# ak110/object_detector

Measured on AMD Instinct MI355X. Metric: images_per_sec, higher is better.
Workload: dtype f16

## Files before the change

object_detector_amd/csrc/conv_8ph.hip:

```cpp
#include "conv_common.h"

namespace {

constexpr int E_BN = 256, E_BK = 64;
constexpr int E_REGION = 128 * 128;
constexpr int E_BUF = 4 * E_REGION;
constexpr int E_ALO = 0, E_AHI = E_REGION, E_BLO = 2 * E_REGION, E_BHI = 3 * E_REGION;

struct TapWalk {
  int c0, tap, tapoff, dx;
  int sel_tap;
};

constexpr unsigned E_OOB = 0x80000000u;

template <int MT, int NF = 4, bool KEEP = false>
static __device__ __forceinline__ void e8_epilogue_direct(const ConvKP& p, f32x4 (&acc)[MT][NF], int m0w, int n0w, int l15,
                                                          int lq, f16x8 (*keep)[NF / 2] = nullptr, int mrows = MT * 16,
                                                          const float* pre_sc = nullptr, const float* pre_bi = nullptr) {
  unsigned pb[MT], ppix[MT];
#pragma unroll
  for (int i = 0; i < MT; ++i) {
    const int m = m0w + i * 16 + l15;
    pb[i] = (unsigned)m / (unsigned)p.HoWo;
    ppix[i] = (unsigned)m - pb[i] * (unsigned)p.HoWo;
  }
#pragma unroll
  for (int pr = 0; pr < NF / 2; ++pr) {
    const int n = n0w + (2 * pr + (lq & 1)) * 16 + (lq >> 1) * 8;
    const bool nok = n < p.Cout;
    float sc[8], bi[8];
    if (pre_sc) {
#pragma unroll
      for (int e = 0; e < 8; ++e) {
        sc[e] = pre_sc[e];
        bi[e] = pre_bi[e];
      }
    } else {
      const f32x4 s0 = *(const f32x4*)(p.scale + n), s1 = *(const f32x4*)(p.scale + n + 4);
      const f32x4 b0 = *(const f32x4*)(p.bias + n), b1 = *(const f32x4*)(p.bias + n + 4);
#pragma unroll
      for (int e = 0; e < 4; ++e) {
        sc[e] = s0[e];
        sc[4 + e] = s1[e];
        bi[e] = b0[e];
        bi[4 + e] = b1[e];
      }
    }
    f16x8 rv[MT];
#pragma unroll
    for (int i = 0; i < MT; ++i) {
      const int m = m0w + i * 16 + l15;
      f16x8 r = {0, 0, 0, 0, 0, 0, 0, 0};
      if (nok && m < p.M && p.res_mode != OD_RES_NONE) {
        long long roff;
        if (p.res_mode == OD_RES_SAME) {
          roff = (long long)m * p.Cout + n;
        } else {
          const unsigned ho = ppix[i] / (unsigned)p.Wo, wo = ppix[i] - ho * (unsigned)p.Wo;
          roff = ((long long)(pb[i] * (unsigned)(p.Ho >> 1) + (ho >> 1)) * (p.Wo >> 1) + (wo >> 1)) * p.Cout + n;
        }
        r = *(const f16x8*)(p.res + roff);
      }
      rv[i] = r;
    }
#pragma unroll
    for (int i = 0; i < MT; ++i) {
      const int m = m0w + i * 16 + l15;
      const bool ok = nok && m < p.M && i * 16 + l15 < mrows;
      float v[8];
#pragma unroll
      for (int e = 0; e < 4; ++e) {
        float a = acc[i][2 * pr][e], bq = acc[i][2 * pr + 1][e];
        od_permlane16_swap(a, bq);
        v[e] = a;
        v[4 + e] = bq;
      }
#pragma unroll
      for (int e = 0; e < 8; ++e) v[e] = v[e] * sc[e] + bi[e];
      if (p.act == OD_ACT_LEAKY) {
#pragma unroll
        for (int e = 0; e < 8; ++e) v[e] = od_leaky(v[e], p.alpha);
      } else if (p.act == OD_ACT_ELU) {
#pragma unroll
        for (int e = 0; e < 8; ++e) v[e] = v[e] > 0.f ? v[e] : p.alpha * od_expm1_fast(v[e]);
      }
      if (p.res_mode != OD_RES_NONE) {
#pragma unroll
        for (int e = 0; e < 8; ++e) v[e] += (float)rv[i][e];
      }
      if (ok) {
        const long long ooff = (long long)pb[i] * p.obs + (long long)ppix[i] * p.ops + n;
        if (p.out_f32) {
          float* o = (float*)p.out + ooff;
          *(f32x4*)o = f32x4{v[0], v[1], v[2], v[3]};
          *(f32x4*)(o + 4) = f32x4{v[4], v[5], v[6], v[7]};
        } else {
          f16x8 h;
#pragma unroll
          for (int e = 0; e < 8; ++e) h[e] = (f16)v[e];
          *(f16x8*)((f16*)p.out + ooff) = h;
        }
      }
      if (KEEP) {
        f16x8 h;
#pragma unroll
        for (int e = 0; e < 8; ++e) h[e] = (f16)v[e];
        keep[i][pr] = h;
      }
    }
  }
}

template <int KS, int MF1, bool PW = false, bool SEG = false>
__global__ __launch_bounds__(512, 2) void od_conv_8ph(ConvKP p_in) {
  constexpr int MF0 = 4, MT = MF0 + MF1, WROWS = MT * 16, BM = 2 * WROWS;
  extern __shared__ __attribute__((aligned(16))) char smem[];
  const int tid = threadIdx.x;
  const int lane = tid & 63;
  const int wave = __builtin_amdgcn_readfirstlane(tid >> 6);
  const int wr = wave >> 2, wc = wave & 3;
  const int l15 = lane & 15, lq = lane >> 4;

  int logical;
  {
    const int nt = p_in.mtiles * p_in.ntiles;
    const int pid = p_in.splitk > 1 ? (int)blockIdx.x / p_in.splitk : (int)blockIdx.x;
    const int q = nt >> 3, r = nt & 7, xcd = pid & 7, loc = pid >> 3;
    logical = (xcd < r ? xcd * (q + 1) : r * (q + 1) + (xcd - r) * q) + loc;
  }
  int tm = logical / p_in.ntiles;
  const int tn = logical - tm * p_in.ntiles;
  ConvKP p_seg;
  if (SEG) p_seg = p_in;
  if (SEG && p_in.nseg > 1) {
    int sg = 0;
    if (tm >= p_in.seg_tile0[1]) sg = 1;
    if (p_in.nseg > 2 && tm >= p_in.seg_tile0[2]) sg = 2;
    tm -= p_in.seg_tile0[sg];
    p_seg.x = p_in.seg_x[sg];
    p_seg.out = p_in.seg_out[sg];
    p_seg.H = p_seg.Ho = p_in.seg_H[sg];
    p_seg.W = p_seg.Wo = p_in.seg_W[sg];
    p_seg.HoWo = p_seg.H * p_seg.W;
    p_seg.M = p_in.seg_M[sg];
    p_seg.x_bytes = (unsigned)p_seg.M * (unsigned)p_in.Cin * 2u;
    if (p_in.obs == 0) p_seg.obs = (long long)p_seg.HoWo * p_in.Cout;
  }
  const ConvKP& p = SEG ? p_seg : p_in;
  const int m0 = tm * BM, n0 = tn * E_BN;
  const int nk_all = p.Ktot / E_BK;
  const int ks0 = p.splitk > 1 ? ((int)blockIdx.x % p.splitk) * p.steps_per_split : 0;
  const int nk = p.splitk > 1 ? min(p.steps_per_split, nk_all - ks0) : nk_all;
  if (nk <= 0) return;

  const int rr = tid >> 3;
  const int lc = (tid & 7) ^ (rr & 7);
  int a_base[2][2];
  unsigned a_vmask[2][2];
  unsigned a_sel[2][2];
#pragma unroll
  for (int s = 0; s < 2; ++s)
#pragma unroll
    for (int j = 0; j < 2; ++j) {
      const int m = m0 + j * WROWS + s * 64 + rr;
      a_vmask[s][j] = 0u;
      a_base[s][j] = 0;
      if (m < p.M && (s == 0 || rr < MF1 * 16)) {
        const unsigned b = (unsigned)m / (unsigned)p.HoWo;
        const unsigned pix = (unsigned)m - b * (unsigned)p.HoWo;
        const unsigned ho = pix / (unsigned)p.Wo;
        const unsigned wo = pix - ho * (unsigned)p.Wo;
        const int hi0 = (int)ho * p.stride - p.pad, wi0 = (int)wo * p.stride - p.pad;
        a_base[s][j] = ((((int)b * p.H + hi0 + p.pad) * p.W + wi0 + p.pad) * p.Cin + lc * 8) * 2;
#pragma unroll
        for (int t = 0; t < KS * KS; ++t) {
          const int hi = hi0 + t / KS, wi = wi0 + t % KS;
          if ((unsigned)hi < (unsigned)p.H && (unsigned)wi < (unsigned)p.W) a_vmask[s][j] |= 1u << t;
        }
      }
    }
  int w_off[2][2];
#pragma unroll
  for (int s = 0; s < 2; ++s)
#pragma unroll
    for (int j = 0; j < 2; ++j) {
      const int n = n0 + (2 * j + (rr >> 5)) * 64 + s * 32 + (rr & 31);
      w_off[s][j] = (n * p.Kstride + lc * 8 + ks0 * E_BK) * 2;
    }
  const __amdgpu_buffer_rsrc_t rs_x = __builtin_amdgcn_make_buffer_rsrc(
      (void*)(p.x - (long long)p.pad * (p.W + 1) * p.Cin), 0, (int)(p.x_bytes + (unsigned)(p.pad * (p.W + 1) * p.Cin * 2)),
      0x00020000);
  const __amdgpu_buffer_rsrc_t rs_w = __builtin_amdgcn_make_buffer_rsrc((void*)p.w, 0, (int)p.w_bytes, 0x00020000);
  auto blds16 = [&](const __amdgpu_buffer_rsrc_t& rs, unsigned voff, int soff, char* lptr) {
    __builtin_amdgcn_raw_ptr_buffer_load_lds(rs, (__attribute__((address_space(3))) void*)lptr, 16, (int)voff, soff, 0, 0);
  };

  auto walk_init = [&](TapWalk& w, int kt) {
    const int k0 = kt * E_BK;
    if (KS == 3) {
      w.sel_tap = -1;
      w.tap = k0 / p.Cin;
      w.c0 = k0 - w.tap * p.Cin;
      const int dy = w.tap / 3;
      w.dx = w.tap - dy * 3;
      w.tapoff = (dy * p.W + w.dx) * p.Cin;
    } else {
      w.sel_tap = -1;
      w.tap = 0;
      w.c0 = k0;
      w.dx = 0;
      w.tapoff = 0;
    }
  };
  auto walk_next = [&](TapWalk& w) {
    w.c0 += E_BK;
    if (KS == 3 && w.c0 >= p.Cin) {
      w.c0 = 0;
      ++w.tap;
      if (++w.dx == 3) {
        w.dx = 0;
        w.tapoff += (p.W - 2) * p.Cin;
      } else {
        w.tapoff += p.Cin;
      }
    }
  };
  TapWalk walk_lo, walk_hi;
  walk_init(walk_lo, ks0);
  walk_init(walk_hi, ks0);

  char* const piece = smem + wave * 1024;
  auto stage_a = [&](int s, TapWalk& w, int buf) {
    const int koff = w.tapoff + w.c0;
    char* dst = piece + buf * E_BUF + (s ? E_AHI : E_ALO);
    if (w.sel_tap != w.tap) {
      w.sel_tap = w.tap;
#pragma unroll
      for (int j = 0; j < 2; ++j) a_sel[s][j] = ((a_vmask[s][j] >> w.tap) & 1u) ? (unsigned)a_base[s][j] : E_OOB;
    }
#pragma unroll
    for (int j = 0; j < 2; ++j) blds16(rs_x, a_sel[s][j], koff * 2, dst + j * 8192);
    walk_next(w);
  };
  auto stage_b = [&](int s, int t, int buf) {
    char* dst = piece + buf * E_BUF + (s ? E_BHI : E_BLO);
#pragma unroll
    for (int j = 0; j < 2; ++j) blds16(rs_w, (unsigned)w_off[s][j], t * (E_BK * 2), dst + j * 8192);
  };

  const int w2buf = ((nk - 1) & 1) ^ 1;
  const __amdgpu_buffer_rsrc_t rs_w2 =
      __builtin_amdgcn_make_buffer_rsrc((void*)(PW ? p.w2 : p.w), 0, (int)(PW ? p.w2_bytes : p.w_bytes), 0x00020000);
  auto stage_w2 = [&](int ks) {
#pragma unroll
    for (int h = 0; h < 2; ++h)
      blds16(rs_w2, (unsigned)(((h * 64 + rr) * p.K2stride + lc * 8) * 2), ks * (E_BK * 2),
             piece + w2buf * E_BUF + ks * E_REGION + h * 8192);
  };

  f32x4 acc[MT][4];
#pragma unroll
  for (int i = 0; i < MT; ++i)
#pragma unroll
    for (int j = 0; j < 4; ++j) acc[i][j] = f32x4{0.f, 0.f, 0.f, 0.f};

  stage_a(0, walk_lo, 0);
  stage_b(0, 0, 0);
  stage_b(1, 0, 0);
  stage_a(1, walk_hi, 0);
  if (nk > 1) {
    stage_a(0, walk_lo, 1);
    stage_b(0, 1, 1);
    wait_vmcnt<8>();
  } else {
    wait_vmcnt<0>();
  }
  __builtin_amdgcn_s_barrier();

  const int fa = (wr * 64 + l15) * 128 + ((lq ^ (l15 & 7)) * 16);
  const int fb = (wc * 32 + l15) * 128 + ((lq ^ (l15 & 7)) * 16);

  f16x8 xa[MF0][2], wlo[2][2], whi[2][2];
  auto ldf = [&](f16x8& dst, const char* src) { dst = *(const f16x8*)src; };
  auto mma = [&](f32x4& c, const f16x8& a, const f16x8& b) {
    c = __builtin_amdgcn_mfma_f32_16x16x32_f16(a, b, c, 0, 0, 0);
  };

  auto L0 = [&](int t) {
    const char* cur = smem + (t & 1) * E_BUF;
#pragma unroll
    for (int f = 0; f < 2; ++f)
#pragma unroll
      for (int kh = 0; kh < 2; ++kh) ldf(wlo[f][kh], cur + E_BLO + ((fb + f * 2048) ^ (kh * 64)));
#pragma unroll
    for (int f = 0; f < MF0; ++f)
#pragma unroll
      for (int kh = 0; kh < 2; ++kh) ldf(xa[f][kh], cur + E_ALO + ((fa + f * 2048) ^ (kh * 64)));
    if (t + 1 < nk) {
      stage_b(1, t + 1, (t & 1) ^ 1);
      wait_vmcnt<8>();
    } else if (PW) {
      stage_w2(0);
      wait_vmcnt<2>();
    } else {
      wait_vmcnt<0>();
    }
  };
  auto L1 = [&](int t) {
    const char* cur = smem + (t & 1) * E_BUF;
#pragma unroll
    for (int f = 0; f < 2; ++f)
#pragma unroll
      for (int kh = 0; kh < 2; ++kh) ldf(whi[f][kh], cur + E_BHI + ((fb + f * 2048) ^ (kh * 64)));
    if (t + 1 < nk) {
      stage_a(1, walk_hi, (t & 1) ^ 1);
      wait_vmcnt<8>();
    } else if (PW) {
      stage_w2(1);
    } else {
      wait_vmcnt<0>();
    }
  };
  auto L2 = [&](int t) {
    const char* cur = smem + (t & 1) * E_BUF;
#pragma unroll
    for (int f = 0; f < MF1; ++f)
#pragma unroll
      for (int kh = 0; kh < 2; ++kh) ldf(xa[f][kh], cur + E_AHI + ((fa + f * 2048) ^ (kh * 64)));
    if (t + 2 < nk) stage_a(0, walk_lo, t & 1);
    if (PW && t + 1 == nk) stage_w2(2);
  };
  auto L3 = [&](int t) {
    if (t + 2 < nk) {
      stage_b(0, t + 2, t & 1);
      wait_vmcnt<8>();
    } else if (PW && t + 1 == nk) {
      stage_w2(3);
    } else {
      wait_vmcnt<0>();
    }
  };
  auto M = [&](int ph) {
    __builtin_amdgcn_s_setprio(1);
#pragma unroll
    for (int kh = 0; kh < 2; ++kh)
#pragma unroll
      for (int i = 0; i < ((ph < 2) ? MF0 : MF1); ++i)
#pragma unroll
        for (int j = 0; j < 2; ++j) {
          if (ph == 0) mma(acc[i][j], wlo[j][kh], xa[i][kh]);
          if (ph == 1) mma(acc[i][2 + j], whi[j][kh], xa[i][kh]);
          if (ph == 2) mma(acc[MF0 + i][2 + j], whi[j][kh], xa[i][kh]);
          if (ph == 3) mma(acc[MF0 + i][j], wlo[j][kh], xa[i][kh]);
        }
    __builtin_amdgcn_s_setprio(0);
  };

  if (wr == 0) {
    for (int t = 0; t < nk; ++t) {
      L0(t);
      M(0);
      __builtin_amdgcn_s_barrier();
      L1(t);
      M(1);
      __builtin_amdgcn_s_barrier();
      L2(t);
      M(2);
      __builtin_amdgcn_s_barrier();
      L3(t);
      M(3);
      __builtin_amdgcn_s_barrier();
    }
  } else {
    L0(0);
    __builtin_amdgcn_s_barrier();
    for (int t = 0; t < nk; ++t) {
      M(0);
      L1(t);
      __builtin_amdgcn_s_barrier();
      M(1);
      L2(t);
      __builtin_amdgcn_s_barrier();
      M(2);
      L3(t);
      __builtin_amdgcn_s_barrier();
      M(3);
      if (t + 1 < nk) {
        L0(t + 1);
        __builtin_amdgcn_s_barrier();
      }
    }
  }
  __syncthreads();

  if (PW) {
    const int rg = wave >> 2, cg = wave & 3;
    float sc2[8], bi2[8];
    {
      const int n2 = cg * 32 + (lq & 1) * 16 + (lq >> 1) * 8;
      const f32x4 s0 = *(const f32x4*)(p.scale2 + n2), s1 = *(const f32x4*)(p.scale2 + n2 + 4);
      const f32x4 b0 = *(const f32x4*)(p.bias2 + n2), b1 = *(const f32x4*)(p.bias2 + n2 + 4);
#pragma unroll
      for (int e = 0; e < 4; ++e) {
        sc2[e] = s0[e];
        sc2[4 + e] = s1[e];
        bi2[e] = b0[e];
        bi2[4 + e] = b1[e];
      }
    }
    f16x8 ykeep[MT][2];
    od_mfma_results_ready();
    e8_epilogue_direct<MT, 4, true>(p, acc, m0 + wr * WROWS, n0 + wc * 64, l15, lq, ykeep);
    ConvKP p2 = p;
    p2.scale = p.scale2;
    p2.bias = p.bias2;
    p2.act = p.act2;
    p2.alpha = p.alpha2;
    p2.res_mode = OD_RES_NONE;
    p2.out = (void*)p.out2;
    p2.out_f32 = 0;
    p2.Cout = p.Cout2;
    p2.obs = (long long)p.HoWo * p.Cout2;
    p2.ops = p.Cout2;
    char* const ybuf = smem + (w2buf ^ 1) * E_BUF;
    const char* const wbuf = smem + w2buf * E_BUF;
    const int fy = (rg * 64 + l15) * 128 + ((lq ^ (l15 & 7)) * 16);
    const int fw = (cg * 32 + l15) * 128 + ((lq ^ (l15 & 7)) * 16);
#pragma unroll
    for (int half = 0; half < 2; ++half) {
      if (wr == half) {
#pragma unroll
        for (int i = 0; i < MT; ++i)
#pragma unroll
          for (int pr = 0; pr < 2; ++pr) {
            const int row = i * 16 + l15;
            const int chunk = (2 * pr + (lq & 1)) * 2 + (lq >> 1);
            *(f16x8*)(ybuf + wc * E_REGION + row * 128 + ((chunk ^ (row & 7)) * 16)) = ykeep[i][pr];
          }
      }
      asm volatile("s_waitcnt lgkmcnt(0)" ::: "memory");
      __builtin_amdgcn_s_barrier();
      f32x4 acc2[4][2];
#pragma unroll
      for (int i = 0; i < 4; ++i)
#pragma unroll
        for (int f = 0; f < 2; ++f) acc2[i][f] = f32x4{0.f, 0.f, 0.f, 0.f};
#pragma unroll
      for (int ks = 0; ks < 4; ++ks)
#pragma unroll
        for (int kh = 0; kh < 2; ++kh) {
          f16x8 wf[2], yf[4];
#pragma unroll
          for (int f = 0; f < 2; ++f) wf[f] = *(const f16x8*)(wbuf + ks * E_REGION + ((fw + f * 2048) ^ (kh * 64)));
#pragma unroll
          for (int i = 0; i < 4; ++i) yf[i] = *(const f16x8*)(ybuf + ks * E_REGION + ((fy + i * 2048) ^ (kh * 64)));
#pragma unroll
          for (int i = 0; i < 4; ++i)
#pragma unroll
            for (int f = 0; f < 2; ++f) acc2[i][f] = __builtin_amdgcn_mfma_f32_16x16x32_f16(wf[f], yf[i], acc2[i][f], 0, 0, 0);
        }
      od_mfma_results_ready();
      e8_epilogue_direct<4, 2>(p2, acc2, m0 + half * WROWS + rg * 64, cg * 32, l15, lq, nullptr, WROWS - rg * 64, sc2, bi2);
      if (half == 0) {
        asm volatile("s_waitcnt lgkmcnt(0)" ::: "memory");
        __builtin_amdgcn_s_barrier();
      }
    }
  } else if (p.splitk > 1) {
    conv_epilogue<E_BN, 2, 4, MT, 4, 512>(p, smem, acc, m0, n0, tid, wr, wc, l15, lq);
  } else {
    od_mfma_results_ready();
    e8_epilogue_direct<MT>(p, acc, m0 + wr * WROWS, n0 + wc * 64, l15, lq);
  }
}

struct E8Entry {
  int BM;
  const void* k1;
  const char* name1;
  const void* k1pw;
  const void* k3pw;
  const char* name1pw;
  const char* name3pw;
  const void* k3seg;
  const char* name3seg;
};
#define OD_E8(MF1)                                                                                                   \
  {                                                                                                                  \
    32 * (4 + MF1), (const void*)&od_conv_8ph<1, MF1>, "od_conv_8ph<1, " #MF1 ", false, false>",                     \
        (const void*)&od_conv_8ph<1, MF1, true>, (const void*)&od_conv_8ph<3, MF1, true>,                            \
        "od_conv_8ph<1, " #MF1 ", true, false>", "od_conv_8ph<3, " #MF1 ", true, false>",                            \
        (const void*)&od_conv_8ph<3, MF1, false, true>, "od_conv_8ph<3, " #MF1 ", false, true>"                      \
  }
const E8Entry g_e8[] = {OD_E8(4), OD_E8(3), OD_E8(2), OD_E8(1)};
constexpr int kNumE8 = sizeof(g_e8) / sizeof(g_e8[0]);

}

int od_conv_8ph_num_cfgs() { return kNumE8; }

long od_conv_8ph_tiles(int idx, int M, int Cout) { return (long)od_ceil_div(M, g_e8[idx].BM) * od_ceil_div(Cout, E_BN); }
double od_conv_8ph_tile_cost(int idx, int nk) { return 13.0 + 1.78 * nk * (0.5 + 0.0625 * (g_e8[idx].BM / 32)); }

bool od_conv_8ph_can_fuse_pointwise(const ConvKP& p) { return p.splitk == 1 && p.Cout == E_BN && p.Cout2 == 128; }

bool od_conv_8ph_select(int idx, const ConvKP& p, int ksize, ConvKernelInfo* info) {
  if (idx < 0 || idx >= kNumE8) return false;
  if ((p.Cin & 63) != 0 || p.tconv) return false;
  if (p.x_bytes >= 0x7F000000u || p.w_bytes >= 0x7F000000u || p.x_bytes == 0) return false;
  const E8Entry& e = g_e8[idx];
  const bool pw = p.w2 != nullptr;
  if (p.nseg > 1 && (ksize != 3 || pw || p.stride != 1 || p.res_mode != OD_RES_NONE)) return false;
  const size_t epi = (size_t)(e.BM / 2) * (E_BN + 4) * 4;
  *info = {ksize == 1 ? (pw ? e.k1pw : e.k1) : (pw ? e.k3pw : e.k3seg),
           ksize == 1 ? (pw ? e.name1pw : e.name1) : (pw ? e.name3pw : e.name3seg),
           e.BM, E_BN, E_BK, 512, epi > (size_t)2 * E_BUF ? epi : (size_t)2 * E_BUF};
  return true;
}
```

object_detector_amd/csrc/conv_common.h:

```cpp
#pragma once
#include "common.h"

struct ConvKP {
  const f16* x;
  const f16* w;
  const float* scale;
  const float* bias;
  const f16* res;
  void* out;
  const f16* zero;
  int H, W, Cin, Ho, Wo, Cout;
  int stride, pad;
  int Kstride, Ktot, M, HoWo;
  int act;
  float alpha;
  int res_mode, out_f32;
  long long obs, ops;
  int mtiles, ntiles;
  int splitk, steps_per_split;
  float* ws;
  int Mq;
  int tconv, Hs, Ws;
  unsigned x_bytes, w_bytes;
  float* stats;
  const f16* w2;
  const float* scale2;
  const float* bias2;
  f16* out2;
  int Cout2, act2;
  float alpha2;
  unsigned w2_bytes;
  int K2stride;
  int nseg;
  int seg_tile0[4];
  const f16* seg_x[3];
  void* seg_out[3];
  int seg_H[3], seg_W[3], seg_M[3];
};

static __device__ __forceinline__ void glds16(const void* gptr, void* lptr) {
  __builtin_amdgcn_global_load_lds((const __attribute__((address_space(1))) void*)gptr,
                                   (__attribute__((address_space(3))) void*)lptr, 16, 0, 0);
}

static __device__ __forceinline__ float od_expm1_fast(float v) {
  const float poly = v * (1.f + v * (0.5f + v * (1.f / 6 + v * (1.f / 24 + v * (1.f / 120 + v * (1.f / 720))))));
  return v > -0.25f ? poly : __expf(v) - 1.f;
}

static __device__ __forceinline__ void od_permlane16_swap(float& a, float& b) {
  asm volatile("s_nop 1\n\tv_permlane16_swap_b32 %0, %1\n\ts_nop 1" : "+v"(a), "+v"(b));
}
static __device__ __forceinline__ void od_mfma_results_ready() {
  __builtin_amdgcn_sched_barrier(0);
  asm volatile("s_nop 15\n\ts_nop 15" ::: "memory");
  __builtin_amdgcn_sched_barrier(0);
}

static __device__ __forceinline__ float od_leaky(float v, float alpha) { return fmaxf(v, v * alpha); }

template <int N>
static __device__ __forceinline__ void wait_vmcnt() {
  asm volatile("s_waitcnt vmcnt(%0)" ::"n"(N) : "memory");
}


static __device__ __forceinline__ int od_tconv_pixel(const ConvKP& p, unsigned m, unsigned BM) {
  const unsigned t = m / BM, r = m - t * BM;
  const unsigned cls = t & 3u, idx = (t >> 2) * BM + r;
  if (idx >= (unsigned)p.Mq) return -1;
  const unsigned HsWs = (unsigned)(p.Hs * p.Ws);
  const unsigned b = idx / HsWs, q = idx - b * HsWs;
  const unsigned i = q / (unsigned)p.Ws, j = q - i * (unsigned)p.Ws;
  return (int)(b * (unsigned)p.HoWo + (2u * i + (cls >> 1)) * (unsigned)p.Wo + 2u * j + (cls & 1u));
}

template <int BN, int WM, int WN, int MT, int NTL, int NT = WM * WN * 64, bool STATS = false>
static __device__ __forceinline__ void conv_epilogue(const ConvKP& p, char* smem, f32x4 (&acc)[MT][NTL], int m0, int n0,
                                                     int tid, int wm, int wn, int l15, int lq) {
  constexpr int WTM = MT * 16, WTN = NTL * 16, SLD = BN + 4;
  float* stg = (float*)smem;
  constexpr int CH = BN / 8;
  constexpr int RPP = NT / CH;
  const int c8 = (tid % CH) * 8;
  const int n = n0 + c8;
  float sc[8], bi[8];
  if (!STATS) {
    const f32x4 s0 = *(const f32x4*)(p.scale + n), s1 = *(const f32x4*)(p.scale + n + 4);
    const f32x4 b0 = *(const f32x4*)(p.bias + n), b1 = *(const f32x4*)(p.bias + n + 4);
#pragma unroll
    for (int e = 0; e < 4; ++e) {
      sc[e] = s0[e];
      sc[4 + e] = s1[e];
      bi[e] = b0[e];
      bi[4 + e] = b1[e];
    }
  }
  float st0[STATS ? 8 : 1], st1[STATS ? 8 : 1];
  if (STATS) {
#pragma unroll
    for (int e = 0; e < 8; ++e) st0[e] = st1[e] = 0.f;
  }
  constexpr int NPASS = (WTM + RPP - 1) / RPP;
  constexpr bool RAGGED = (WTM % RPP) != 0;
  f16x8 resv[WM][NPASS];
  if (p.res_mode != OD_RES_NONE && p.splitk <= 1) {
#pragma unroll
    for (int wr = 0; wr < WM; ++wr)
#pragma unroll
      for (int ps = 0; ps < NPASS; ++ps) {
        int m = m0 + wr * WTM + ps * RPP + tid / CH;
        f16x8 r = {0, 0, 0, 0, 0, 0, 0, 0};
        if (RAGGED && ps * RPP + tid / CH >= WTM) m = p.M;
        if (p.tconv && m < p.M) m = od_tconv_pixel(p, (unsigned)m, WM * MT * 16);
        if (m >= 0 && m < p.M && n < p.Cout) {
          long long roff;
          if (p.res_mode == OD_RES_SAME) {
            roff = (long long)m * p.Cout + n;
          } else {
            const unsigned b = (unsigned)m / (unsigned)p.HoWo;
            const unsigned pix = (unsigned)m - b * (unsigned)p.HoWo;
            const unsigned ho = pix / (unsigned)p.Wo, wo = pix - ho * (unsigned)p.Wo;
            roff = ((long long)(b * (unsigned)(p.Ho >> 1) + (ho >> 1)) * (p.Wo >> 1) + (wo >> 1)) * p.Cout + n;
          }
          r = *(const f16x8*)(p.res + roff);
        }
        resv[wr][ps] = r;
      }
  }
#pragma unroll
  for (int wr = 0; wr < WM; ++wr) {
    if (wm == wr) {
#pragma unroll
      for (int j = 0; j < NTL; ++j) {
        const int nl = wn * WTN + j * 16 + lq * 4;
#pragma unroll
        for (int i = 0; i < MT; ++i) *(f32x4*)(stg + (i * 16 + l15) * SLD + nl) = acc[i][j];
      }
    }
    __syncthreads();
    if (p.splitk > 1) {
      float* slab = p.ws + (long long)((int)blockIdx.x % p.splitk) * p.M * p.Cout;
#pragma unroll
      for (int ps = 0; ps < NPASS; ++ps) {
        const int row = ps * RPP + tid / CH;
        const int m = (RAGGED && row >= WTM) ? p.M : m0 + wr * WTM + row;
        if (m < p.M && n < p.Cout) {
          float* o = slab + (long long)m * p.Cout + n;
          *(f32x4*)o = *(const f32x4*)(stg + row * SLD + c8);
          *(f32x4*)(o + 4) = *(const f32x4*)(stg + row * SLD + c8 + 4);
        }
      }
      if (wr + 1 < WM) __syncthreads();
      continue;
    }
#pragma unroll
    for (int ps = 0; ps < NPASS; ++ps) {
      const int row = ps * RPP + tid / CH;
      int m = (RAGGED && row >= WTM) ? p.M : m0 + wr * WTM + row;
      if (p.tconv && m < p.M) m = od_tconv_pixel(p, (unsigned)m, WM * MT * 16);
      if (m >= 0 && m < p.M && n < p.Cout) {
        const f32x4 v0 = *(const f32x4*)(stg + row * SLD + c8);
        const f32x4 v1 = *(const f32x4*)(stg + row * SLD + c8 + 4);
        float v[8] = {v0[0], v0[1], v0[2], v0[3], v1[0], v1[1], v1[2], v1[3]};
        if (!STATS) {
#pragma unroll
          for (int e = 0; e < 8; ++e) v[e] = v[e] * sc[e] + bi[e];
        }
        if (STATS) {
        } else if (p.act == OD_ACT_LEAKY) {
#pragma unroll
          for (int e = 0; e < 8; ++e) v[e] = od_leaky(v[e], p.alpha);
        } else if (p.act == OD_ACT_ELU) {
#pragma unroll
          for (int e = 0; e < 8; ++e) v[e] = v[e] > 0.f ? v[e] : p.alpha * od_expm1_fast(v[e]);
        }
        if (!STATS && p.res_mode != OD_RES_NONE) {
#pragma unroll
          for (int e = 0; e < 8; ++e) v[e] += (float)resv[wr][ps][e];
        }
        const unsigned b = (unsigned)m / (unsigned)p.HoWo;
        const unsigned pix = (unsigned)m - b * (unsigned)p.HoWo;
        const long long ooff = (long long)b * p.obs + (long long)pix * p.ops + n;
        if (p.out_f32) {
          float* o = (float*)p.out + ooff;
          *(f32x4*)o = f32x4{v[0], v[1], v[2], v[3]};
          *(f32x4*)(o + 4) = f32x4{v[4], v[5], v[6], v[7]};
        } else {
          f16x8 h;
#pragma unroll
          for (int e = 0; e < 8; ++e) h[e] = (f16)v[e];
          *(f16x8*)((f16*)p.out + ooff) = h;
          if (STATS) {
#pragma unroll
            for (int e = 0; e < 8; ++e) {
              const float q = (float)h[e];
              st0[e] += q;
              st1[e] += q * q;
            }
          }
        }
      }
    }
    if (wr + 1 < WM) __syncthreads();
  }
  if (STATS) {
    static_assert(CH == 8 || CH == 16 || CH == 32, "BN must be 64, 128 or 256");
#pragma unroll
    for (int off = CH; off < 64; off <<= 1) {
#pragma unroll
      for (int e = 0; e < 8; ++e) {
        st0[e] += __shfl_xor(st0[e], off, 64);
        st1[e] += __shfl_xor(st1[e], off, 64);
      }
    }
    __syncthreads();
    float* red = (float*)smem;
    const int wv = tid >> 6, ln = tid & 63;
    if (ln < CH) {
#pragma unroll
      for (int e = 0; e < 8; ++e) {
        red[(wv * CH + ln) * 16 + e] = st0[e];
        red[(wv * CH + ln) * 16 + 8 + e] = st1[e];
      }
    }
    __syncthreads();
    if (tid < CH && n < p.Cout) {
      float a[8], b[8];
#pragma unroll
      for (int e = 0; e < 8; ++e) a[e] = b[e] = 0.f;
      for (int w2 = 0; w2 < NT / 64; ++w2) {
#pragma unroll
        for (int e = 0; e < 8; ++e) {
          a[e] += red[(w2 * CH + tid) * 16 + e];
          b[e] += red[(w2 * CH + tid) * 16 + 8 + e];
        }
      }
      float* row = p.stats + (long long)(m0 / (WM * WTM)) * 2 * p.Cout;
#pragma unroll
      for (int e = 0; e < 8; ++e) {
        row[n + e] = a[e];
        row[p.Cout + n + e] = b[e];
      }
    }
  }
}

struct ConvKernelInfo {
  const void* fn;
  const char* name;
  int BM, BN, BK, threads;
  size_t lds;
};

int od_conv_igemm_num_cfgs();
bool od_conv_igemm_select(int cfg, int ksize, int Cin, bool want_stats, ConvKernelInfo* info);
int od_conv_finish_prepare(const ConvKP& p, od_launches* L);
int od_conv_8ph_num_cfgs();
long od_conv_8ph_tiles(int idx, int M, int Cout);
double od_conv_8ph_tile_cost(int idx, int nk);
bool od_conv_8ph_can_fuse_pointwise(const ConvKP& p);
bool od_conv_8ph_select(int idx, const ConvKP& p, int ksize, ConvKernelInfo* info);
bool od_tconv_small_supported(const od_conv_desc* d);
int od_tconv_small_prepare(od_ctx* ctx, const od_conv_desc* d, od_launches* L);
bool od_conv_rdirect_supported(const od_conv_desc* d);
int od_conv_rdirect_prepare(od_ctx* ctx, const od_conv_desc* d, od_launches* L);
bool od_conv_stream3_supported(const od_conv_desc* d);
int od_conv_stream3_prepare(od_ctx* ctx, const od_conv_desc* d, od_launches* L);
```

object_detector_amd/csrc/conv_dispatch.hip:

```cpp
#include <string.h>

#include "conv_common.h"

namespace {

int pick_cfg(const od_ctx* ctx, int M, int Cin, int Cout, int ksize, bool e8_ok, bool throughput) {
  const int cus = ctx->num_cu;
  const int cfg_e8 = od_conv_igemm_num_cfgs();
  const bool spec_ok = (Cin % 64) == 0;
  if (Cout <= 64) return (ksize == 3 && od_ceil_div(M, 128) >= 8 * cus) ? 1 : 3;
  const long t128 = (long)od_ceil_div(M, 128) * od_ceil_div(Cout, 128);
  if (ksize == 1) {
    if (!spec_ok) return 3;
    if (M <= 4096) return (M >= 2048 && Cin >= 512) ? 6 : 3;
    if (M <= 16384) return 7;
    if (Cout < 256) return 3;
    if (t128 < cus) return 4;
  }
  if (!spec_ok) return t128 >= 2L * cus ? 0 : 2;
  const int nk = od_ceil_div(ksize * ksize * Cin, 64);
  if (throughput && e8_ok && ksize == 3 && Cout >= 192 && M >= 2048) {
    double best = t128 >= cus ? t128 * (7.5 + 1.07 * nk) * 0.5 : t128 * (10.0 + 0.55 * nk);
    int pick = t128 >= cus ? 4 : (Cout <= 256 ? 7 : 5);
    for (int i = 0; i < od_conv_8ph_num_cfgs(); ++i) {
      const long tiles = od_conv_8ph_tiles(i, M, Cout);
      if (tiles * 3 < cus) continue;
      const double c = (double)tiles * od_conv_8ph_tile_cost(i, nk);
      if (c < 0.95 * best) {
        best = c / 0.95;
        pick = cfg_e8 + i;
      }
    }
    return pick;
  }
  if (t128 >= cus) {
    if (Cout == 128) return 2;
    const double c13 = (double)od_ceil_div((int)t128, 2 * cus) * (7.5 + 1.07 * nk);
    double best = 0.93 * c13;
    int pick = 4;
    for (int i = 0; e8_ok && i < od_conv_8ph_num_cfgs(); ++i) {
      const double c = (double)((od_conv_8ph_tiles(i, M, Cout) + cus - 1) / cus) * od_conv_8ph_tile_cost(i, nk);
      if (c < best) {
        best = c;
        pick = cfg_e8 + i;
      }
    }
    return pick;
  }
  if (Cout <= 256) return M < 2048 ? 3 : 7;
  return (M >= 2048 && 2 * t128 <= cus) ? 7 : 5;
}

int conv_describe(const od_ctx* ctx, const od_conv_desc* d, bool want_stats, od_conv_desc* v, ConvKP* kp) {
  if (d && d->nseg > 1) {
    OD_REQUIRE(d->nseg <= 3, "od_conv2d_fwd: nseg %d > 3", d->nseg);
    OD_REQUIRE(d->ksize == 3 && d->stride == 1 && d->res_mode == OD_RES_NONE && !d->w2 && !want_stats && !d->transposed,
               "od_conv2d_fwd: a grouped launch (nseg > 1) is a 3x3 stride-1 layer without residual / w2 / bn_partials / "
               "transposed mode");
    for (int i = 0; i < d->nseg; ++i)
      OD_REQUIRE(d->seg_x[i] && d->seg_out[i] && d->seg_H[i] > 0 && d->seg_W[i] > 0, "od_conv2d_fwd: segment %d is incomplete", i);
  }
  OD_REQUIRE(ctx && d, "od_conv2d_fwd: null ctx/desc");
  *v = *d;
  const bool grouped = d->nseg > 1;
  if (grouped) {
    v->x = d->seg_x[0];
    v->out = d->seg_out[0];
    v->H = d->seg_H[0];
    v->W = d->seg_W[0];
  }
  d = v;
  OD_REQUIRE(d->x && d->w && d->scale && d->bias && d->out, "od_conv2d_fwd: null tensor");
  OD_REQUIRE(d->ksize == 1 || d->ksize == 3, "od_conv2d_fwd: ksize %d unsupported", d->ksize);
  OD_REQUIRE(d->stride == 1 || d->stride == 2, "od_conv2d_fwd: stride %d unsupported", d->stride);
  OD_REQUIRE(d->B > 0 && d->H > 0 && d->W > 0 && d->Cin > 0 && d->Cout > 0, "od_conv2d_fwd: bad dims");
  OD_REQUIRE(d->Cin % 8 == 0 && d->Cout % 8 == 0, "od_conv2d_fwd: Cin/Cout must be multiples of 8 (got %d/%d)",
             d->Cin, d->Cout);
  OD_REQUIRE(d->res_mode == OD_RES_NONE || d->res, "od_conv2d_fwd: res_mode set but res is null");
  OD_REQUIRE(d->act >= OD_ACT_LINEAR && d->act <= OD_ACT_ELU, "od_conv2d_fwd: bad act");
  OD_REQUIRE(d->act != OD_ACT_LEAKY || (d->alpha >= 0.f && d->alpha <= 1.f), "od_conv2d_fwd: leaky slope must be in [0, 1]");
  ConvKP& p = *kp;
  p.pad = d->ksize / 2;
  p.tconv = d->transposed != 0;
  if (p.tconv)
    OD_REQUIRE(d->ksize == 3 && d->stride == 2 && d->Cin % 64 == 0,
               "od_conv2d_fwd: transposed mode is the backward-data of a 3x3 stride-2 conv (Cin %% 64 == 0)");
  p.H = p.tconv ? 2 * d->H : d->H;
  p.W = p.tconv ? 2 * d->W : d->W;
  p.stride = p.tconv ? 1 : d->stride;
  p.Hs = d->H;
  p.Ws = d->W;
  p.Ho = (p.H + 2 * p.pad - d->ksize) / p.stride + 1;
  p.Wo = (p.W + 2 * p.pad - d->ksize) / p.stride + 1;
  if (d->res_mode == OD_RES_UP2)
    OD_REQUIRE(p.Ho % 2 == 0 && p.Wo % 2 == 0, "od_conv2d_fwd: OD_RES_UP2 needs even output size");
  const long long M64 = (long long)d->B * p.Ho * p.Wo;
  OD_REQUIRE(M64 * d->Cout < (1LL << 31) && (long long)d->B * d->H * d->W * d->Cin < (1LL << 31),
             "od_conv2d_fwd: tensor too large for 32-bit element offsets");
  p.HoWo = p.Ho * p.Wo;
  long long Mg = 0;
  for (int i = 0; grouped && i < d->nseg; ++i) Mg += (long long)d->B * d->seg_H[i] * d->seg_W[i];
  OD_REQUIRE(!grouped || Mg * d->Cout < (1LL << 31), "od_conv2d_fwd: grouped launch too large for 32-bit element offsets");
  p.M = grouped ? (int)Mg : (int)M64;
  p.nseg = grouped ? d->nseg : 0;

  if (want_stats)
    OD_REQUIRE(!p.tconv && d->out_dtype == OD_DT_F16 && d->act == OD_ACT_LINEAR && d->res_mode == OD_RES_NONE,
               "od_conv2d_fwd: bn_partials needs the raw convolution (f16 output, no activation, no residual, no transposed "
               "gather; scale / bias are NOT applied)");
  if (d->w2) {
    OD_REQUIRE(d->scale2 && d->bias2 && d->out2 && d->Cout2 > 0 && d->Cout2 % 8 == 0,
               "od_conv2d_fwd: w2 needs scale2, bias2, out2 and Cout2 (a multiple of 8)");
    OD_REQUIRE(d->act2 >= OD_ACT_LINEAR && d->act2 <= OD_ACT_ELU, "od_conv2d_fwd: bad act2");
    OD_REQUIRE(d->act2 != OD_ACT_LEAKY || (d->alpha2 >= 0.f && d->alpha2 <= 1.f), "od_conv2d_fwd: leaky slope (alpha2) must be in [0, 1]");
    OD_REQUIRE(d->out_dtype == OD_DT_F16 && !p.tconv && !want_stats && d->Cout % 8 == 0 &&
                   (d->out_batch_stride == 0 || d->out_batch_stride == (long long)p.HoWo * d->Cout) &&
                   (d->out_pix_stride == 0 || d->out_pix_stride == d->Cout),
               "od_conv2d_fwd: w2 (the consuming pointwise layer) needs a dense f16 output of the first layer");
  }
  p.x = (const f16*)d->x;
  p.w = (const f16*)d->w;
  p.scale = d->scale;
  p.bias = d->bias;
  p.res = (const f16*)d->res;
  p.out = d->out;
  p.zero = (const f16*)ctx->zero_page;
  p.Cin = d->Cin;
  p.Cout = d->Cout;
  p.Ktot = d->ksize * d->ksize * d->Cin;
  p.Kstride = od_round_up(p.Ktot, 64);
  p.act = d->act;
  p.alpha = d->alpha;
  p.res_mode = d->res_mode;
  p.out_f32 = d->out_dtype == OD_DT_F32;
  p.stats = d->bn_partials;
  p.w2 = nullptr;
  p.scale2 = d->scale2;
  p.bias2 = d->bias2;
  p.out2 = (f16*)d->out2;
  p.Cout2 = d->Cout2;
  p.act2 = d->act2;
  p.alpha2 = d->alpha2;
  p.K2stride = od_round_up(d->Cout, 64);
  p.w2_bytes = (unsigned)((long long)od_round_up(d->Cout2 > 0 ? d->Cout2 : 1, 256) * p.K2stride * 2);
  p.x_bytes = (unsigned)((long long)d->B * d->H * d->W * d->Cin * 2);
  p.w_bytes = (unsigned)((long long)od_round_up(d->Cout, 256) * p.Kstride * 2);
  p.obs = d->out_batch_stride ? d->out_batch_stride : (long long)p.HoWo * d->Cout;
  p.ops = d->out_pix_stride ? d->out_pix_stride : d->Cout;
  p.splitk = 1;
  p.steps_per_split = 0;
  p.ws = (float*)d->splitk_workspace;
  return OD_OK;
}

int conv_choose_cfg(const od_ctx* ctx, const od_conv_desc* d, const ConvKP& p, bool want_stats, int* cfg_out) {
  int cfg = d->tile_cfg;
  if (cfg < 0)
    cfg = pick_cfg(ctx, p.M, d->Cin, d->Cout, d->ksize, !want_stats && !p.tconv && (long long)p.x_bytes < 0x7F000000LL, cfg == -2);
  const int cfg_e8 = od_conv_igemm_num_cfgs();
  OD_REQUIRE(cfg < cfg_e8 + od_conv_8ph_num_cfgs(), "od_conv2d_fwd: tile_cfg %d out of range", cfg);
  OD_REQUIRE(!(want_stats && cfg >= cfg_e8), "od_conv2d_fwd: bn_partials is supported by the table kernels only (tile_cfg %d)", cfg);
  OD_REQUIRE(!p.tconv || cfg < cfg_e8, "od_conv2d_fwd: transposed mode runs on the table kernels only (tile_cfg %d)", cfg);
  *cfg_out = cfg;
  return OD_OK;
}

int conv_select(int cfg, const od_conv_desc* d, const ConvKP& p, bool want_stats, ConvKernelInfo* k) {
  const int cfg_e8 = od_conv_igemm_num_cfgs();
  if (cfg >= cfg_e8) {
    if (od_conv_8ph_select(cfg - cfg_e8, p, d->ksize, k)) return OD_OK;
    od_set_error("od_conv2d_fwd: tile_cfg %d (8-phase kernel) needs Cin %% 64 == 0 and no transposed gather", cfg);
    return OD_ERR_INVALID;
  }
  if (od_conv_igemm_select(cfg, d->ksize, d->Cin, want_stats, k)) return OD_OK;
  od_set_error("od_conv2d_fwd: tile_cfg %d needs Cin %% %d == 0 for 3x3 (Cin = %d); use cfg 0-3", cfg, k->BK, d->Cin);
  return OD_ERR_INVALID;
}

void conv_tile_kp(const od_conv_desc* d, const ConvKernelInfo& k, ConvKP* kp) {
  ConvKP& p = *kp;
  p.mtiles = od_ceil_div(p.M, k.BM);
  if (p.nseg > 1) {
    int t0 = 0;
    for (int i = 0; i < 3; ++i) {
      const bool used = i < d->nseg;
      p.seg_tile0[i] = t0;
      p.seg_x[i] = used ? (const f16*)d->seg_x[i] : nullptr;
      p.seg_out[i] = used ? d->seg_out[i] : nullptr;
      p.seg_H[i] = used ? d->seg_H[i] : 0;
      p.seg_W[i] = used ? d->seg_W[i] : 0;
      p.seg_M[i] = d->B * p.seg_H[i] * p.seg_W[i];
      t0 += od_ceil_div(p.seg_M[i], k.BM);
    }
    p.seg_tile0[3] = t0;
    p.mtiles = t0;
    if (!d->out_batch_stride) p.obs = 0;
  }
  p.Mq = 0;
  if (p.tconv) {
    p.Mq = p.M / 4;
    p.mtiles = 4 * od_ceil_div(p.Mq, k.BM);
    p.M = p.mtiles * k.BM;
  }
  p.ntiles = od_ceil_div(d->Cout, k.BN);
}

int conv_prepare(od_ctx* ctx, const od_conv_desc* desc, bool want_stats, od_launches* L) {
  od_conv_desc v;
  ConvKP p;
  if (int rc = conv_describe(ctx, desc, want_stats, &v, &p)) return rc;
  const od_conv_desc* d = &v;
  const bool grouped = p.nseg > 1;
  if (d->tile_cfg < 0 && !want_stats && !grouped) {
    if (p.tconv && od_tconv_small_supported(d)) return od_tconv_small_prepare(ctx, d, L);
    if (od_conv_rdirect_supported(d)) return od_conv_rdirect_prepare(ctx, d, L);
    if (!p.tconv && od_conv_stream3_supported(d)) return od_conv_stream3_prepare(ctx, d, L);
  }
  int cfg;
  if (int rc = conv_choose_cfg(ctx, d, p, want_stats, &cfg)) return rc;
  const bool use_e8 = cfg >= od_conv_igemm_num_cfgs();
  if (grouped && !(use_e8 && d->Cin % 64 == 0)) {
    od_conv_desc q = *d;
    q.nseg = 0;
    for (int i = 0; i < d->nseg; ++i) {
      q.x = d->seg_x[i];
      q.out = d->seg_out[i];
      q.H = d->seg_H[i];
      q.W = d->seg_W[i];
      if (int rc = conv_prepare(ctx, &q, false, L)) return rc;
    }
    return OD_OK;
  }
  ConvKernelInfo k;
  if (int rc = conv_select(cfg, d, p, want_stats, &k)) return rc;
  conv_tile_kp(d, k, &p);
  if (d->bn_partials) {
    const long long need = (long long)p.mtiles * 2 * d->Cout * 4;
    if (d->bn_partials_bytes < need) {
      od_set_error("od_conv2d_fwd: bn_partials holds %lld bytes, %d rows x 2 x %d channels need %lld", (long long)d->bn_partials_bytes,
                   p.mtiles, d->Cout, need);
      return OD_ERR_WORKSPACE;
    }
  }
  if (d->splitk_workspace && d->splitk != 1 && !p.tconv && !want_stats && !grouped) {
    const int cus = ctx->num_cu;
    const int tiles = p.mtiles * p.ntiles;
    const int nk = od_ceil_div(p.Ktot, k.BK);
    constexpr int thr_mul = 8;
    constexpr int tgt_mul = 1;
    int sk = d->splitk > 1 ? d->splitk : ((tiles * thr_mul <= cus && nk >= 8) ? od_ceil_div(tgt_mul * cus / 2, tiles) : 1);
    if (sk > nk / 4) sk = nk / 4;
    const long long slab_bytes = (long long)p.M * d->Cout * 4;
    if ((long long)sk * slab_bytes > (long long)d->splitk_workspace_bytes) sk = (int)(d->splitk_workspace_bytes / slab_bytes);
    if (sk > 1) {
      p.steps_per_split = od_ceil_div(nk, sk);
      p.splitk = od_ceil_div(nk, p.steps_per_split);
    }
  }
  if (d->w2 && use_e8 && od_conv_8ph_can_fuse_pointwise(p)) {
    p.w2 = (const f16*)d->w2;
    if (int rc = conv_select(cfg, d, p, want_stats, &k)) return rc;
  }
  if (int rc = od_ensure_lds(ctx, k.fn, k.lds)) return rc;
  const size_t launch_lds = (use_e8 && p.splitk <= 1 && k.lds > (size_t)128 * 1024) ? (size_t)128 * 1024 : k.lds;
  if (int rc = od_add_launch(L, {k.name, od_issue_kp, k.fn, dim3(p.mtiles * p.ntiles * p.splitk), dim3(k.threads), launch_lds}, p))
    return rc;
  if (p.splitk > 1)
    if (int rc = od_conv_finish_prepare(p, L)) return rc;
  if (!d->w2 || p.w2) return OD_OK;
  od_conv_desc q;
  memset(&q, 0, sizeof(q));
  q.x = d->out;
  q.w = d->w2;
  q.scale = d->scale2;
  q.bias = d->bias2;
  q.out = d->out2;
  q.B = d->B;
  q.H = p.Ho;
  q.W = p.Wo;
  q.Cin = d->Cout;
  q.Cout = d->Cout2;
  q.ksize = 1;
  q.stride = 1;
  q.act = d->act2;
  q.alpha = d->alpha2;
  q.res_mode = OD_RES_NONE;
  q.out_dtype = OD_DT_F16;
  q.tile_cfg = d->tile_cfg < 0 ? d->tile_cfg : -1;
  q.splitk = d->splitk;
  q.splitk_workspace = d->splitk_workspace;
  q.splitk_workspace_bytes = d->splitk_workspace_bytes;
  return conv_prepare(ctx, &q, false, L);
}

}

extern "C" int od_conv_num_tile_cfgs(void) { return od_conv_igemm_num_cfgs() + od_conv_8ph_num_cfgs(); }

extern "C" int od_conv_weight_dims(int cout, int cin, int ksize, int* cout_pad, int* kpad) {
  OD_REQUIRE(cout > 0 && cin > 0 && (ksize == 1 || ksize == 3), "od_conv_weight_dims: bad dims");
  if (cout_pad) *cout_pad = od_round_up(cout, 256);
  if (kpad) *kpad = od_round_up(ksize * ksize * cin, 64);
  return OD_OK;
}

int od_conv_prepare(od_ctx* ctx, const od_conv_desc* d, od_launches* L) {
  return conv_prepare(ctx, d, d && d->bn_partials, L);
}

extern "C" int od_conv2d_fwd(od_ctx* ctx, const od_conv_desc* d, void* stream) {
  return od_prepare_issue(stream, od_conv_prepare, ctx, d);
}

extern "C" int od_conv2d_fwd_bn_rows(od_ctx* ctx, const od_conv_desc* d) {
  od_conv_desc v;
  ConvKP p;
  ConvKernelInfo k;
  int cfg;
  if (conv_describe(ctx, d, true, &v, &p) || conv_choose_cfg(ctx, &v, p, true, &cfg) || conv_select(cfg, &v, p, true, &k)) return -1;
  conv_tile_kp(&v, k, &p);
  return p.mtiles;
}

extern "C" int od_conv2d_bwd_data(od_ctx* ctx, const void* dz, const void* w_bwd, const void* dx_accumulate, void* dx, int B,
                                  int Ho, int Wo, int Cin, int Cout, int ksize, int stride, void* stream) {
  OD_REQUIRE(ctx && dz && w_bwd && dx, "od_conv2d_bwd_data: null argument");
  OD_REQUIRE(Cin > 0 && Cin <= 2048, "od_conv2d_bwd_data: Cin out of range (1..2048)");
  od_conv_desc d;
  memset(&d, 0, sizeof(d));
  d.x = dz;
  d.w = w_bwd;
  d.scale = ctx->ones;
  d.bias = (const float*)ctx->zero_page;
  d.res = dx_accumulate;
  d.res_mode = dx_accumulate ? OD_RES_SAME : OD_RES_NONE;
  d.out = dx;
  d.B = B;
  d.H = Ho;
  d.W = Wo;
  d.Cin = Cout;
  d.Cout = Cin;
  d.ksize = ksize;
  d.stride = stride;
  d.act = OD_ACT_LINEAR;
  d.out_dtype = OD_DT_F16;
  d.tile_cfg = -1;
  d.transposed = stride == 2;
  d.splitk = 1;
  return od_conv2d_fwd(ctx, &d, stream);
}
```

object_detector_amd/csrc/conv_mfma.hip:

```cpp
#include <stdlib.h>
#include <string.h>

#include "conv_common.h"

namespace {

template <int BM, int BN, int BK, int STAGES, int WM, int WN, int SPEC = 0>
struct ConvCfg {
  static constexpr int NT = WM * WN * 64;
  static constexpr int NTHREADS = NT * (SPEC ? 2 : 1);
  static constexpr int CPR = BK / 8;
  static constexpr int RPR = NT / CPR;
  static constexpr int AR = BM / RPR, BR = BN / RPR;
  static constexpr int ROWB = BK * 2;
  static constexpr int A_BYTES = BM * ROWB, B_BYTES = BN * ROWB, STAGE_BYTES = A_BYTES + B_BYTES;
  static constexpr int WTM = BM / WM, WTN = BN / WN;
  static constexpr int MT = WTM / 16, NTL = WTN / 16;
  static constexpr int SLD = BN + 4;
  static constexpr int PIPE_BYTES = STAGES * STAGE_BYTES;
  static constexpr int EPI_BYTES = WTM * SLD * 4;
  static constexpr int LDS_BYTES = PIPE_BYTES > EPI_BYTES ? PIPE_BYTES : EPI_BYTES;
  static constexpr int LOADS = AR + BR;
  static_assert(BM % RPR == 0 && BN % RPR == 0, "tile must be a whole number of DMA rounds");
  static_assert(BK == 32 || BK == 64, "BK");
  static_assert(LOADS * (STAGES - 2 > 0 ? STAGES - 2 : 0) <= 63, "vmcnt field");
};

template <int BM, int BN, int BK, int STAGES, int WM, int WN, int KS, int MINW, bool UNI, int SPEC, bool STATS = false>
__global__ __launch_bounds__(WM* WN * 64 * (SPEC ? 2 : 1), MINW) void od_conv_igemm(ConvKP p) {
  using Cf = ConvCfg<BM, BN, BK, STAGES, WM, WN, SPEC>;
  constexpr int NT = Cf::NT, AR = Cf::AR, BR = Cf::BR, RPR = Cf::RPR, ROWB = Cf::ROWB;
  constexpr int WTM = Cf::WTM, WTN = Cf::WTN, MT = Cf::MT, NTL = Cf::NTL;

  extern __shared__ __attribute__((aligned(16))) char smem[];

  const int tid_all = threadIdx.x;
  const int lane = tid_all & 63;
  const int wave_all = __builtin_amdgcn_readfirstlane(tid_all >> 6);
  const bool is_loader = SPEC ? (wave_all >= WM * WN) : true;
  const bool is_consumer = SPEC ? (wave_all < WM * WN) : true;
  const int tid = SPEC ? (tid_all & (NT - 1)) : tid_all;
  const int wave = SPEC ? (wave_all >= WM * WN ? wave_all - WM * WN : wave_all) : wave_all;
  const int l15 = lane & 15, lq = lane >> 4;

  int logical;
  {
    const int nt = p.mtiles * p.ntiles;
    const int pid = p.splitk > 1 ? (int)blockIdx.x / p.splitk : (int)blockIdx.x;
    const int q = nt >> 3, r = nt & 7, xcd = pid & 7, loc = pid >> 3;
    logical = (xcd < r ? xcd * (q + 1) : r * (q + 1) + (xcd - r) * q) + loc;
  }
  const int tm = logical / p.ntiles, tn = logical - tm * p.ntiles;
  const int m0 = tm * BM, n0 = tn * BN;
  const int nk_all = (p.Ktot + BK - 1) / BK;
  const int ks0 = p.splitk > 1 ? ((int)blockIdx.x % p.splitk) * p.steps_per_split : 0;
  int nk = p.splitk > 1 ? min(p.steps_per_split, nk_all - ks0) : nk_all;
  if (nk <= 0) return;

  int rr, lc, piece_off;
  if (BK == 64) {
    rr = tid >> 3;
    lc = (tid & 7) ^ (rr & 7);
    piece_off = wave * 8 * ROWB;
  } else {
    rr = wave * 16 + (lane & 15);
    lc = lane >> 4;
    piece_off = wave * 16 * ROWB;
  }
  int a_base[AR], a_hi0[AR], a_wi0[AR], a_b[AR];
  unsigned a_vmask[AR];
#pragma unroll
  for (int rd = 0; rd < AR; ++rd) {
    int m = m0 + rd * RPR + rr;
    a_vmask[rd] = 0u;
    if (p.tconv && m < p.M) m = od_tconv_pixel(p, (unsigned)m, BM);
    if (m >= 0 && m < p.M) {
      const unsigned b = (unsigned)m / (unsigned)p.HoWo;
      const unsigned pix = (unsigned)m - b * (unsigned)p.HoWo;
      const unsigned ho = pix / (unsigned)p.Wo;
      const unsigned wo = pix - ho * (unsigned)p.Wo;
      a_hi0[rd] = (int)ho * p.stride - p.pad;
      a_wi0[rd] = (int)wo * p.stride - p.pad;
      a_base[rd] = (((int)b * p.H + a_hi0[rd]) * p.W + a_wi0[rd]) * p.Cin + lc * 8;
      a_b[rd] = (int)b;
#pragma unroll
      for (int t = 0; t < KS * KS; ++t) {
        const int hi = a_hi0[rd] + t / KS, wi = a_wi0[rd] + t % KS;
        bool ok = (unsigned)hi < (unsigned)p.H && (unsigned)wi < (unsigned)p.W;
        if (p.tconv) ok = ok && !((hi | wi) & 1);
        if (ok) a_vmask[rd] |= 1u << t;
      }
    } else {
      a_hi0[rd] = -(1 << 24);
      a_wi0[rd] = 0;
      a_base[rd] = 0;
      a_b[rd] = 0;
    }
  }
  const f16* wrow = p.w + (long long)(n0 + rr) * p.Kstride + lc * 8;

  unsigned tmask = 0x1FFu;
  if (UNI && KS == 3 && p.tconv && p.splitk <= 1) {
    unsigned um = 0u;
#pragma unroll
    for (int rd = 0; rd < AR; ++rd) um |= a_vmask[rd];
    for (int off = 32; off; off >>= 1) um |= (unsigned)__shfl_xor((int)um, off, 64);
    unsigned* sh = (unsigned*)smem;
    if (tid_all == 0) *sh = 0u;
    __syncthreads();
    if (lane == 0) atomicOr(sh, um);
    __syncthreads();
    tmask = (unsigned)__builtin_amdgcn_readfirstlane((int)*sh);
    __syncthreads();
    nk = __builtin_popcount(tmask) * (p.Cin / BK);
  }

  int ld_k0 = ks0 * BK, ld_c0 = ld_k0, ld_tap = 0, ld_tapoff = 0, ld_dx = 0, ld_dy = 0;
  if (UNI && KS == 3) {
    ld_tap = ld_k0 / p.Cin;
    ld_c0 = ld_k0 - ld_tap * p.Cin;
    if (tmask != 0x1FFu && tmask != 0u) {
      ld_tap = __builtin_ctz(tmask);
      ld_c0 = 0;
      ld_k0 = ld_tap * p.Cin;
    }
    ld_dy = ld_tap / 3;
    ld_dx = ld_tap - ld_dy * 3;
    ld_tapoff = (ld_dy * p.W + ld_dx) * p.Cin;
  }

  constexpr int NX = AR + BR;
  f16x8 rtmp[SPEC == 2 ? NX : 1];
  char* rdst[SPEC == 2 ? NX : 1];
  int rn = 0;
  auto xfer = [&](const f16* src, char* lds_piece) {
    if (SPEC == 2) {
      rtmp[rn] = *(const f16x8*)src;
      rdst[rn] = lds_piece + lane * 16;
      ++rn;
    } else {
      glds16(src, lds_piece);
    }
  };
  auto stage = [&](int buf) {
    rn = 0;
    char* abuf = smem + buf * Cf::STAGE_BYTES + piece_off;
    char* bbuf = abuf + Cf::A_BYTES;
    if (UNI) {
      const bool cvalid = (KS == 3) || (ld_c0 + lc * 8 < p.Cin);
      const int koff = ld_tapoff + ld_c0;
#pragma unroll
      for (int rd = 0; rd < AR; ++rd) {
        const bool ok = cvalid && ((a_vmask[rd] >> ld_tap) & 1u);
        const f16* src;
        if (KS == 3 && p.tconv) {
          const int u = (a_hi0[rd] + ld_dy) >> 1, v = (a_wi0[rd] + ld_dx) >> 1;
          src = ok ? p.x + (((a_b[rd] * p.Hs + u) * p.Ws + v) * p.Cin + lc * 8 + ld_c0) : p.zero;
        } else {
          src = ok ? p.x + (a_base[rd] + koff) : p.zero;
        }
        xfer(src, abuf + rd * RPR * ROWB);
      }
    } else {
      const int k = ld_k0 + lc * 8;
      const int tap = k / p.Cin;
      const int dy = tap / 3, dx = tap - dy * 3;
      const int cin = k - tap * p.Cin;
      const bool kvalid = k < p.Ktot;
      const int koff = (dy * p.W + dx) * p.Cin + cin - lc * 8;
#pragma unroll
      for (int rd = 0; rd < AR; ++rd) {
        const int hi = a_hi0[rd] + dy, wi = a_wi0[rd] + dx;
        const bool ok = kvalid && (unsigned)hi < (unsigned)p.H && (unsigned)wi < (unsigned)p.W;
        const f16* src = ok ? p.x + (a_base[rd] + koff) : p.zero;
        xfer(src, abuf + rd * RPR * ROWB);
      }
    }
#pragma unroll
    for (int rd = 0; rd < BR; ++rd) xfer(wrow + (long long)rd * RPR * p.Kstride + ld_k0, bbuf + rd * RPR * ROWB);
    if (SPEC == 2) {
#pragma unroll
      for (int i = 0; i < NX; ++i) *(f16x8*)rdst[i] = rtmp[i];
    }
    ld_k0 += BK;
    if (UNI) {
      ld_c0 += BK;
      if (KS == 3 && ld_c0 >= p.Cin) {
        ld_c0 = 0;
        ++ld_tap;
        if (++ld_dx == 3) {
          ld_dx = 0;
          ++ld_dy;
          ld_tapoff += (p.W - 2) * p.Cin;
        } else {
          ld_tapoff += p.Cin;
        }
        while (ld_tap < 9 && !((tmask >> ld_tap) & 1u)) {
          ++ld_tap;
          ld_k0 += p.Cin;
          if (++ld_dx == 3) {
            ld_dx = 0;
            ++ld_dy;
          }
        }
      }
    }
  };

  const int wm = wave / WN, wn = wave - wm * WN;
  f32x4 acc[MT][NTL];
#pragma unroll
  for (int i = 0; i < MT; ++i)
#pragma unroll
    for (int j = 0; j < NTL; ++j) acc[i][j] = f32x4{0.f, 0.f, 0.f, 0.f};

  if (is_loader) {
#pragma unroll
    for (int s = 0; s < STAGES - 1; ++s)
      if (s < nk) stage(s);
  }

  const int swz = l15 & 7;
  int buf = 0;
  for (int ks = 0; ks < nk; ++ks) {
    if (is_loader) {
      if (STAGES > 2 && ks + (STAGES - 2) < nk)
        wait_vmcnt<Cf::LOADS*(STAGES > 2 ? STAGES - 2 : 0)>();
      else
        wait_vmcnt<0>();
    }
    if (SPEC == 2) asm volatile("s_waitcnt lgkmcnt(0)" ::: "memory");
    __builtin_amdgcn_s_barrier();
    {
      const int nxt = ks + STAGES - 1;
      int nb = buf + STAGES - 1;
      if (nb >= STAGES) nb -= STAGES;
      if (is_loader && nxt < nk) stage(nb);
    }
    const char* abuf = smem + buf * Cf::STAGE_BYTES;
    const char* bbuf = abuf + Cf::A_BYTES;
    __builtin_amdgcn_s_setprio(1);
    if (is_consumer)
#pragma unroll
    for (int kh = 0; kh < BK / 32; ++kh) {
      f16x8 xa[MT], wb[NTL];
      if (BK == 64) {
        const int coff = ((kh * 4 + lq) ^ swz) * 16;
#pragma unroll
        for (int i = 0; i < MT; ++i) xa[i] = *(const f16x8*)(abuf + (wm * WTM + i * 16 + l15) * ROWB + coff);
#pragma unroll
        for (int j = 0; j < NTL; ++j) wb[j] = *(const f16x8*)(bbuf + (wn * WTN + j * 16 + l15) * ROWB + coff);
      } else {
        const int coff = lq * 256 + l15 * 16;
#pragma unroll
        for (int i = 0; i < MT; ++i) xa[i] = *(const f16x8*)(abuf + (wm * WTM + i * 16) * ROWB + coff);
#pragma unroll
        for (int j = 0; j < NTL; ++j) wb[j] = *(const f16x8*)(bbuf + (wn * WTN + j * 16) * ROWB + coff);
      }
#pragma unroll
      for (int i = 0; i < MT; ++i)
#pragma unroll
        for (int j = 0; j < NTL; ++j)
          acc[i][j] = __builtin_amdgcn_mfma_f32_16x16x32_f16(wb[j], xa[i], acc[i][j], 0, 0, 0);
    }
    __builtin_amdgcn_s_setprio(0);
    if (++buf == STAGES) buf = 0;
  }
  __syncthreads();

  conv_epilogue<BN, WM, WN, MT, NTL, Cf::NTHREADS, STATS>(p, smem, acc, m0, n0, tid_all, is_consumer ? wm : -1, wn, l15, lq);
}

__global__ __launch_bounds__(256) void od_conv_finish(ConvKP p) {
  const long long nvec = (long long)p.M * (p.Cout >> 3);
  const int C8 = p.Cout >> 3;
  for (long long i = (long long)blockIdx.x * 256 + threadIdx.x; i < nvec; i += (long long)gridDim.x * 256) {
    const int m = (int)(i / C8), n = (int)(i - (long long)m * C8) * 8;
    const float* wsp = p.ws + (long long)m * p.Cout + n;
    const long long slab = (long long)p.M * p.Cout;
    float v[8] = {0.f, 0.f, 0.f, 0.f, 0.f, 0.f, 0.f, 0.f};
    for (int sidx = 0; sidx < p.splitk; ++sidx) {
      const f32x4 a0 = *(const f32x4*)(wsp + sidx * slab), a1 = *(const f32x4*)(wsp + sidx * slab + 4);
#pragma unroll
      for (int e = 0; e < 4; ++e) {
        v[e] += a0[e];
        v[4 + e] += a1[e];
      }
    }
#pragma unroll
    for (int e = 0; e < 8; ++e) {
      v[e] = v[e] * p.scale[n + e] + p.bias[n + e];
      if (p.act == OD_ACT_LEAKY) v[e] = od_leaky(v[e], p.alpha);
      else if (p.act == OD_ACT_ELU) v[e] = v[e] > 0.f ? v[e] : p.alpha * od_expm1_fast(v[e]);
    }
    const unsigned b = (unsigned)m / (unsigned)p.HoWo;
    const unsigned pix = (unsigned)m - b * (unsigned)p.HoWo;
    if (p.res_mode != OD_RES_NONE) {
      long long roff;
      if (p.res_mode == OD_RES_SAME) {
        roff = (long long)m * p.Cout + n;
      } else {
        const unsigned ho = pix / (unsigned)p.Wo, wo = pix - ho * (unsigned)p.Wo;
        roff = ((long long)(b * (unsigned)(p.Ho >> 1) + (ho >> 1)) * (p.Wo >> 1) + (wo >> 1)) * p.Cout + n;
      }
      const f16x8 r = *(const f16x8*)(p.res + roff);
#pragma unroll
      for (int e = 0; e < 8; ++e) v[e] += (float)r[e];
    }
    const long long ooff = (long long)b * p.obs + (long long)pix * p.ops + n;
    if (p.out_f32) {
      float* o = (float*)p.out + ooff;
      *(f32x4*)o = f32x4{v[0], v[1], v[2], v[3]};
      *(f32x4*)(o + 4) = f32x4{v[4], v[5], v[6], v[7]};
    } else {
      f16x8 h;
#pragma unroll
      for (int e = 0; e < 8; ++e) h[e] = (f16)v[e];
      *(f16x8*)((f16*)p.out + ooff) = h;
    }
  }
}

struct TileCfg {
  int BM, BN, BK, threads;
  size_t lds;
  struct { const void* fn; const char* name; } k[3][2];
};

#define OD_K1(BM, BN, BK, ST, WM, WN, KS, MINW, UNI, SPEC, STATS)                                                       \
  {(const void*)&od_conv_igemm<BM, BN, BK, ST, WM, WN, KS, MINW, UNI, SPEC, STATS>,                                     \
   "od_conv_igemm<" #BM ", " #BN ", " #BK ", " #ST ", " #WM ", " #WN ", " #KS ", " #MINW ", " #UNI ", " #SPEC ", " #STATS ">"}
#define OD_K(BM, BN, BK, ST, WM, WN, KS, MINW, UNI, SPEC)                                                              \
  {OD_K1(BM, BN, BK, ST, WM, WN, KS, MINW, UNI, SPEC, false), OD_K1(BM, BN, BK, ST, WM, WN, KS, MINW, UNI, SPEC, true)}
#define OD_NOK(BM, BN, BK, ST, WM, WN, KS, MINW, UNI, SPEC) {}
#define OD_CFG(BM, BN, BK, ST, WM, WN, MINW, SPEC, K3G)                                                                 \
  {BM, BN, BK, WM * WN * 64 * (SPEC + 1), (size_t)ConvCfg<BM, BN, BK, ST, WM, WN, SPEC>::LDS_BYTES,                     \
   {OD_K(BM, BN, BK, ST, WM, WN, 1, MINW, true, SPEC), OD_K(BM, BN, BK, ST, WM, WN, 3, MINW, true, SPEC),               \
    K3G(BM, BN, BK, ST, WM, WN, 3, MINW, false, SPEC)}}

const TileCfg g_cfgs[] = {
    OD_CFG(128, 128, 64, 2, 2, 2, 2, 0, OD_K),
    OD_CFG(128, 64, 64, 2, 2, 2, 2, 0, OD_K),
    OD_CFG(64, 128, 64, 2, 2, 2, 2, 0, OD_K),
    OD_CFG(64, 64, 64, 2, 2, 2, 2, 0, OD_K),
    OD_CFG(128, 128, 64, 2, 2, 2, 4, 1, OD_NOK),
    OD_CFG(128, 128, 64, 3, 2, 2, 2, 1, OD_NOK),
    OD_CFG(64, 64, 64, 4, 2, 2, 2, 0, OD_NOK),
    OD_CFG(64, 128, 64, 3, 2, 2, 4, 1, OD_NOK),
};
constexpr int kNumCfgs = sizeof(g_cfgs) / sizeof(g_cfgs[0]);

}

int od_conv_igemm_num_cfgs() { return kNumCfgs; }

bool od_conv_igemm_select(int cfg, int ksize, int Cin, bool want_stats, ConvKernelInfo* info) {
  if (cfg < 0 || cfg >= kNumCfgs) return false;
  const TileCfg& tc = g_cfgs[cfg];
  const auto& k = tc.k[ksize == 1 ? 0 : ((Cin % tc.BK) == 0 ? 1 : 2)][want_stats];
  *info = {k.fn, k.name, tc.BM, tc.BN, tc.BK, tc.threads, tc.lds};
  return k.fn != nullptr;
}

int od_conv_finish_prepare(const ConvKP& p, od_launches* L) {
  const long long nvec = (long long)p.M * (p.Cout / 8);
  long long fb = (nvec + 255) / 256;
  if (fb > 2048) fb = 2048;
  return od_add_launch(L, {"od_conv_finish", od_issue_kp, (const void*)&od_conv_finish, dim3((unsigned)fb), dim3(256), 0}, p);
}
```

Before: 21570.

## Specialize conv epilogues at compile time by activation/residual mode with 32-bit offsets

Adds an EPI template parameter so conv kernels are instantiated for the common activation, residual and output-type combinations, and the dispatcher picks a specialized kernel per layer. This removes runtime branches on act, res_mode and out_f32 in the epilogue. It also computes a flag that allows 32-bit output offset arithmetic when the output fits. The 8-phase kernel moves into a header with per-MF variant selectors. In exchange there are many more kernel instantiations, which raises compile time and binary size.

```diff
diff --git a/object_detector_amd/csrc/conv_8ph.hip b/object_detector_amd/csrc/conv_8ph.hip
--- a/object_detector_amd/csrc/conv_8ph.hip
+++ b/object_detector_amd/csrc/conv_8ph.hip
@@ -1,499 +1,14 @@
+#include "conv_8ph_tile.h"
 #include "conv_common.h"
 
 namespace {
 
-constexpr int E_BN = 256, E_BK = 64;
-constexpr int E_REGION = 128 * 128;
-constexpr int E_BUF = 4 * E_REGION;
-constexpr int E_ALO = 0, E_AHI = E_REGION, E_BLO = 2 * E_REGION, E_BHI = 3 * E_REGION;
-
-struct TapWalk {
-  int c0, tap, tapoff, dx;
-  int sel_tap;
-};
-
-constexpr unsigned E_OOB = 0x80000000u;
-
-template <int MT, int NF = 4, bool KEEP = false>
-static __device__ __forceinline__ void e8_epilogue_direct(const ConvKP& p, f32x4 (&acc)[MT][NF], int m0w, int n0w, int l15,
-                                                          int lq, f16x8 (*keep)[NF / 2] = nullptr, int mrows = MT * 16,
-                                                          const float* pre_sc = nullptr, const float* pre_bi = nullptr) {
-  unsigned pb[MT], ppix[MT];
-#pragma unroll
-  for (int i = 0; i < MT; ++i) {
-    const int m = m0w + i * 16 + l15;
-    pb[i] = (unsigned)m / (unsigned)p.HoWo;
-    ppix[i] = (unsigned)m - pb[i] * (unsigned)p.HoWo;
-  }
-#pragma unroll
-  for (int pr = 0; pr < NF / 2; ++pr) {
-    const int n = n0w + (2 * pr + (lq & 1)) * 16 + (lq >> 1) * 8;
-    const bool nok = n < p.Cout;
-    float sc[8], bi[8];
-    if (pre_sc) {
-#pragma unroll
-      for (int e = 0; e < 8; ++e) {
-        sc[e] = pre_sc[e];
-        bi[e] = pre_bi[e];
-      }
-    } else {
-      const f32x4 s0 = *(const f32x4*)(p.scale + n), s1 = *(const f32x4*)(p.scale + n + 4);
-      const f32x4 b0 = *(const f32x4*)(p.bias + n), b1 = *(const f32x4*)(p.bias + n + 4);
-#pragma unroll
-      for (int e = 0; e < 4; ++e) {
-        sc[e] = s0[e];
-        sc[4 + e] = s1[e];
-        bi[e] = b0[e];
-        bi[4 + e] = b1[e];
-      }
-    }
-    f16x8 rv[MT];
-#pragma unroll
-    for (int i = 0; i < MT; ++i) {
-      const int m = m0w + i * 16 + l15;
-      f16x8 r = {0, 0, 0, 0, 0, 0, 0, 0};
-      if (nok && m < p.M && p.res_mode != OD_RES_NONE) {
-        long long roff;
-        if (p.res_mode == OD_RES_SAME) {
-          roff = (long long)m * p.Cout + n;
-        } else {
-          const unsigned ho = ppix[i] / (unsigned)p.Wo, wo = ppix[i] - ho * (unsigned)p.Wo;
-          roff = ((long long)(pb[i] * (unsigned)(p.Ho >> 1) + (ho >> 1)) * (p.Wo >> 1) + (wo >> 1)) * p.Cout + n;
-        }
-        r = *(const f16x8*)(p.res + roff);
-      }
-      rv[i] = r;
-    }
-#pragma unroll
-    for (int i = 0; i < MT; ++i) {
-      const int m = m0w + i * 16 + l15;
-      const bool ok = nok && m < p.M && i * 16 + l15 < mrows;
-      float v[8];
-#pragma unroll
-      for (int e = 0; e < 4; ++e) {
-        float a = acc[i][2 * pr][e], bq = acc[i][2 * pr + 1][e];
-        od_permlane16_swap(a, bq);
-        v[e] = a;
-        v[4 + e] = bq;
-      }
-#pragma unroll
-      for (int e = 0; e < 8; ++e) v[e] = v[e] * sc[e] + bi[e];
-      if (p.act == OD_ACT_LEAKY) {
-#pragma unroll
-        for (int e = 0; e < 8; ++e) v[e] = od_leaky(v[e], p.alpha);
-      } else if (p.act == OD_ACT_ELU) {
-#pragma unroll
-        for (int e = 0; e < 8; ++e) v[e] = v[e] > 0.f ? v[e] : p.alpha * od_expm1_fast(v[e]);
-      }
-      if (p.res_mode != OD_RES_NONE) {
-#pragma unroll
-        for (int e = 0; e < 8; ++e) v[e] += (float)rv[i][e];
-      }
-      if (ok) {
-        const long long ooff = (long long)pb[i] * p.obs + (long long)ppix[i] * p.ops + n;
-        if (p.out_f32) {
-          float* o = (float*)p.out + ooff;
-          *(f32x4*)o = f32x4{v[0], v[1], v[2], v[3]};
-          *(f32x4*)(o + 4) = f32x4{v[4], v[5], v[6], v[7]};
-        } else {
-          f16x8 h;
-#pragma unroll
-          for (int e = 0; e < 8; ++e) h[e] = (f16)v[e];
-          *(f16x8*)((f16*)p.out + ooff) = h;
-        }
-      }
-      if (KEEP) {
-        f16x8 h;
-#pragma unroll
-        for (int e = 0; e < 8; ++e) h[e] = (f16)v[e];
-        keep[i][pr] = h;
-      }
-    }
-  }
-}
-
-template <int KS, int MF1, bool PW = false, bool SEG = false>
-__global__ __launch_bounds__(512, 2) void od_conv_8ph(ConvKP p_in) {
-  constexpr int MF0 = 4, MT = MF0 + MF1, WROWS = MT * 16, BM = 2 * WROWS;
-  extern __shared__ __attribute__((aligned(16))) char smem[];
-  const int tid = threadIdx.x;
-  const int lane = tid & 63;
-  const int wave = __builtin_amdgcn_readfirstlane(tid >> 6);
-  const int wr = wave >> 2, wc = wave & 3;
-  const int l15 = lane & 15, lq = lane >> 4;
-
-  int logical;
-  {
-    const int nt = p_in.mtiles * p_in.ntiles;
-    const int pid = p_in.splitk > 1 ? (int)blockIdx.x / p_in.splitk : (int)blockIdx.x;
-    const int q = nt >> 3, r = nt & 7, xcd = pid & 7, loc = pid >> 3;
-    logical = (xcd < r ? xcd * (q + 1) : r * (q + 1) + (xcd - r) * q) + loc;
-  }
-  int tm = logical / p_in.ntiles;
-  const int tn = logical - tm * p_in.ntiles;
-  ConvKP p_seg;
-  if (SEG) p_seg = p_in;
-  if (SEG && p_in.nseg > 1) {
-    int sg = 0;
-    if (tm >= p_in.seg_tile0[1]) sg = 1;
-    if (p_in.nseg > 2 && tm >= p_in.seg_tile0[2]) sg = 2;
-    tm -= p_in.seg_tile0[sg];
-    p_seg.x = p_in.seg_x[sg];
-    p_seg.out = p_in.seg_out[sg];
-    p_seg.H = p_seg.Ho = p_in.seg_H[sg];
-    p_seg.W = p_seg.Wo = p_in.seg_W[sg];
-    p_seg.HoWo = p_seg.H * p_seg.W;
-    p_seg.M = p_in.seg_M[sg];
-    p_seg.x_bytes = (unsigned)p_seg.M * (unsigned)p_in.Cin * 2u;
-    if (p_in.obs == 0) p_seg.obs = (long long)p_seg.HoWo * p_in.Cout;
-  }
-  const ConvKP& p = SEG ? p_seg : p_in;
-  const int m0 = tm * BM, n0 = tn * E_BN;
-  const int nk_all = p.Ktot / E_BK;
-  const int ks0 = p.splitk > 1 ? ((int)blockIdx.x % p.splitk) * p.steps_per_split : 0;
-  const int nk = p.splitk > 1 ? min(p.steps_per_split, nk_all - ks0) : nk_all;
-  if (nk <= 0) return;
-
-  const int rr = tid >> 3;
-  const int lc = (tid & 7) ^ (rr & 7);
-  int a_base[2][2];
-  unsigned a_vmask[2][2];
-  unsigned a_sel[2][2];
-#pragma unroll
-  for (int s = 0; s < 2; ++s)
-#pragma unroll
-    for (int j = 0; j < 2; ++j) {
-      const int m = m0 + j * WROWS + s * 64 + rr;
-      a_vmask[s][j] = 0u;
-      a_base[s][j] = 0;
-      if (m < p.M && (s == 0 || rr < MF1 * 16)) {
-        const unsigned b = (unsigned)m / (unsigned)p.HoWo;
-        const unsigned pix = (unsigned)m - b * (unsigned)p.HoWo;
-        const unsigned ho = pix / (unsigned)p.Wo;
-        const unsigned wo = pix - ho * (unsigned)p.Wo;
-        const int hi0 = (int)ho * p.stride - p.pad, wi0 = (int)wo * p.stride - p.pad;
-        a_base[s][j] = ((((int)b * p.H + hi0 + p.pad) * p.W + wi0 + p.pad) * p.Cin + lc * 8) * 2;
-#pragma unroll
-        for (int t = 0; t < KS * KS; ++t) {
-          const int hi = hi0 + t / KS, wi = wi0 + t % KS;
-          if ((unsigned)hi < (unsigned)p.H && (unsigned)wi < (unsigned)p.W) a_vmask[s][j] |= 1u << t;
-        }
-      }
-    }
-  int w_off[2][2];
-#pragma unroll
-  for (int s = 0; s < 2; ++s)
-#pragma unroll
-    for (int j = 0; j < 2; ++j) {
-      const int n = n0 + (2 * j + (rr >> 5)) * 64 + s * 32 + (rr & 31);
-      w_off[s][j] = (n * p.Kstride + lc * 8 + ks0 * E_BK) * 2;
-    }
-  const __amdgpu_buffer_rsrc_t rs_x = __builtin_amdgcn_make_buffer_rsrc(
-      (void*)(p.x - (long long)p.pad * (p.W + 1) * p.Cin), 0, (int)(p.x_bytes + (unsigned)(p.pad * (p.W + 1) * p.Cin * 2)),
-      0x00020000);
-  const __amdgpu_buffer_rsrc_t rs_w = __builtin_amdgcn_make_buffer_rsrc((void*)p.w, 0, (int)p.w_bytes, 0x00020000);
-  auto blds16 = [&](const __amdgpu_buffer_rsrc_t& rs, unsigned voff, int soff, char* lptr) {
-    __builtin_amdgcn_raw_ptr_buffer_load_lds(rs, (__attribute__((address_space(3))) void*)lptr, 16, (int)voff, soff, 0, 0);
-  };
-
-  auto walk_init = [&](TapWalk& w, int kt) {
-    const int k0 = kt * E_BK;
-    if (KS == 3) {
-      w.sel_tap = -1;
-      w.tap = k0 / p.Cin;
-      w.c0 = k0 - w.tap * p.Cin;
-      const int dy = w.tap / 3;
-      w.dx = w.tap - dy * 3;
-      w.tapoff = (dy * p.W + w.dx) * p.Cin;
-    } else {
-      w.sel_tap = -1;
-      w.tap = 0;
-      w.c0 = k0;
-      w.dx = 0;
-      w.tapoff = 0;
-    }
-  };
-  auto walk_next = [&](TapWalk& w) {
-    w.c0 += E_BK;
-    if (KS == 3 && w.c0 >= p.Cin) {
-      w.c0 = 0;
-      ++w.tap;
-      if (++w.dx == 3) {
-        w.dx = 0;
-        w.tapoff += (p.W - 2) * p.Cin;
-      } else {
-        w.tapoff += p.Cin;
-      }
-    }
-  };
-  TapWalk walk_lo, walk_hi;
-  walk_init(walk_lo, ks0);
-  walk_init(walk_hi, ks0);
-
-  char* const piece = smem + wave * 1024;
-  auto stage_a = [&](int s, TapWalk& w, int buf) {
-    const int koff = w.tapoff + w.c0;
-    char* dst = piece + buf * E_BUF + (s ? E_AHI : E_ALO);
-    if (w.sel_tap != w.tap) {
-      w.sel_tap = w.tap;
-#pragma unroll
-      for (int j = 0; j < 2; ++j) a_sel[s][j] = ((a_vmask[s][j] >> w.tap) & 1u) ? (unsigned)a_base[s][j] : E_OOB;
-    }
-#pragma unroll
-    for (int j = 0; j < 2; ++j) blds16(rs_x, a_sel[s][j], koff * 2, dst + j * 8192);
-    walk_next(w);
-  };
-  auto stage_b = [&](int s, int t, int buf) {
-    char* dst = piece + buf * E_BUF + (s ? E_BHI : E_BLO);
-#pragma unroll
-    for (int j = 0; j < 2; ++j) blds16(rs_w, (unsigned)w_off[s][j], t * (E_BK * 2), dst + j * 8192);
-  };
-
-  const int w2buf = ((nk - 1) & 1) ^ 1;
-  const __amdgpu_buffer_rsrc_t rs_w2 =
-      __builtin_amdgcn_make_buffer_rsrc((void*)(PW ? p.w2 : p.w), 0, (int)(PW ? p.w2_bytes : p.w_bytes), 0x00020000);
-  auto stage_w2 = [&](int ks) {
-#pragma unroll
-    for (int h = 0; h < 2; ++h)
-      blds16(rs_w2, (unsigned)(((h * 64 + rr) * p.K2stride + lc * 8) * 2), ks * (E_BK * 2),
-             piece + w2buf * E_BUF + ks * E_REGION + h * 8192);
-  };
-
-  f32x4 acc[MT][4];
-#pragma unroll
-  for (int i = 0; i < MT; ++i)
-#pragma unroll
-    for (int j = 0; j < 4; ++j) acc[i][j] = f32x4{0.f, 0.f, 0.f, 0.f};
-
-  stage_a(0, walk_lo, 0);
-  stage_b(0, 0, 0);
-  stage_b(1, 0, 0);
-  stage_a(1, walk_hi, 0);
-  if (nk > 1) {
-    stage_a(0, walk_lo, 1);
-    stage_b(0, 1, 1);
-    wait_vmcnt<8>();
-  } else {
-    wait_vmcnt<0>();
-  }
-  __builtin_amdgcn_s_barrier();
-
-  const int fa = (wr * 64 + l15) * 128 + ((lq ^ (l15 & 7)) * 16);
-  const int fb = (wc * 32 + l15) * 128 + ((lq ^ (l15 & 7)) * 16);
-
-  f16x8 xa[MF0][2], wlo[2][2], whi[2][2];
-  auto ldf = [&](f16x8& dst, const char* src) { dst = *(const f16x8*)src; };
-  auto mma = [&](f32x4& c, const f16x8& a, const f16x8& b) {
-    c = __builtin_amdgcn_mfma_f32_16x16x32_f16(a, b, c, 0, 0, 0);
-  };
-
-  auto L0 = [&](int t) {
-    const char* cur = smem + (t & 1) * E_BUF;
-#pragma unroll
-    for (int f = 0; f < 2; ++f)
-#pragma unroll
-      for (int kh = 0; kh < 2; ++kh) ldf(wlo[f][kh], cur + E_BLO + ((fb + f * 2048) ^ (kh * 64)));
-#pragma unroll
-    for (int f = 0; f < MF0; ++f)
-#pragma unroll
-      for (int kh = 0; kh < 2; ++kh) ldf(xa[f][kh], cur + E_ALO + ((fa + f * 2048) ^ (kh * 64)));
-    if (t + 1 < nk) {
-      stage_b(1, t + 1, (t & 1) ^ 1);
-      wait_vmcnt<8>();
-    } else if (PW) {
-      stage_w2(0);
-      wait_vmcnt<2>();
-    } else {
-      wait_vmcnt<0>();
-    }
-  };
-  auto L1 = [&](int t) {
-    const char* cur = smem + (t & 1) * E_BUF;
-#pragma unroll
-    for (int f = 0; f < 2; ++f)
-#pragma unroll
-      for (int kh = 0; kh < 2; ++kh) ldf(whi[f][kh], cur + E_BHI + ((fb + f * 2048) ^ (kh * 64)));
-    if (t + 1 < nk) {
-      stage_a(1, walk_hi, (t & 1) ^ 1);
-      wait_vmcnt<8>();
-    } else if (PW) {
-      stage_w2(1);
-    } else {
-      wait_vmcnt<0>();
-    }
-  };
-  auto L2 = [&](int t) {
-    const char* cur = smem + (t & 1) * E_BUF;
-#pragma unroll
-    for (int f = 0; f < MF1; ++f)
-#pragma unroll
-      for (int kh = 0; kh < 2; ++kh) ldf(xa[f][kh], cur + E_AHI + ((fa + f * 2048) ^ (kh * 64)));
-    if (t + 2 < nk) stage_a(0, walk_lo, t & 1);
-    if (PW && t + 1 == nk) stage_w2(2);
-  };
-  auto L3 = [&](int t) {
-    if (t + 2 < nk) {
-      stage_b(0, t + 2, t & 1);
-      wait_vmcnt<8>();
-    } else if (PW && t + 1 == nk) {
-      stage_w2(3);
-    } else {
-      wait_vmcnt<0>();
-    }
-  };
-  auto M = [&](int ph) {
-    __builtin_amdgcn_s_setprio(1);
-#pragma unroll
-    for (int kh = 0; kh < 2; ++kh)
-#pragma unroll
-      for (int i = 0; i < ((ph < 2) ? MF0 : MF1); ++i)
-#pragma unroll
-        for (int j = 0; j < 2; ++j) {
-          if (ph == 0) mma(acc[i][j], wlo[j][kh], xa[i][kh]);
-          if (ph == 1) mma(acc[i][2 + j], whi[j][kh], xa[i][kh]);
-          if (ph == 2) mma(acc[MF0 + i][2 + j], whi[j][kh], xa[i][kh]);
-          if (ph == 3) mma(acc[MF0 + i][j], wlo[j][kh], xa[i][kh]);
-        }
-    __builtin_amdgcn_s_setprio(0);
-  };
-
-  if (wr == 0) {
-    for (int t = 0; t < nk; ++t) {
-      L0(t);
-      M(0);
-      __builtin_amdgcn_s_barrier();
-      L1(t);
-      M(1);
-      __builtin_amdgcn_s_barrier();
-      L2(t);
-      M(2);
-      __builtin_amdgcn_s_barrier();
-      L3(t);
-      M(3);
-      __builtin_amdgcn_s_barrier();
-    }
-  } else {
-    L0(0);
-    __builtin_amdgcn_s_barrier();
-    for (int t = 0; t < nk; ++t) {
-      M(0);
-      L1(t);
-      __builtin_amdgcn_s_barrier();
-      M(1);
-      L2(t);
-      __builtin_amdgcn_s_barrier();
-      M(2);
-      L3(t);
-      __builtin_amdgcn_s_barrier();
-      M(3);
-      if (t + 1 < nk) {
-        L0(t + 1);
-        __builtin_amdgcn_s_barrier();
-      }
-    }
-  }
-  __syncthreads();
-
-  if (PW) {
-    const int rg = wave >> 2, cg = wave & 3;
-    float sc2[8], bi2[8];
-    {
-      const int n2 = cg * 32 + (lq & 1) * 16 + (lq >> 1) * 8;
-      const f32x4 s0 = *(const f32x4*)(p.scale2 + n2), s1 = *(const f32x4*)(p.scale2 + n2 + 4);
-      const f32x4 b0 = *(const f32x4*)(p.bias2 + n2), b1 = *(const f32x4*)(p.bias2 + n2 + 4);
-#pragma unroll
-      for (int e = 0; e < 4; ++e) {
-        sc2[e] = s0[e];
-        sc2[4 + e] = s1[e];
-        bi2[e] = b0[e];
-        bi2[4 + e] = b1[e];
-      }
-    }
-    f16x8 ykeep[MT][2];
-    od_mfma_results_ready();
-    e8_epilogue_direct<MT, 4, true>(p, acc, m0 + wr * WROWS, n0 + wc * 64, l15, lq, ykeep);
-    ConvKP p2 = p;
-    p2.scale = p.scale2;
-    p2.bias = p.bias2;
-    p2.act = p.act2;
-    p2.alpha = p.alpha2;
-    p2.res_mode = OD_RES_NONE;
-    p2.out = (void*)p.out2;
-    p2.out_f32 = 0;
-    p2.Cout = p.Cout2;
-    p2.obs = (long long)p.HoWo * p.Cout2;
-    p2.ops = p.Cout2;
-    char* const ybuf = smem + (w2buf ^ 1) * E_BUF;
-    const char* const wbuf = smem + w2buf * E_BUF;
-    const int fy = (rg * 64 + l15) * 128 + ((lq ^ (l15 & 7)) * 16);
-    const int fw = (cg * 32 + l15) * 128 + ((lq ^ (l15 & 7)) * 16);
-#pragma unroll
-    for (int half = 0; half < 2; ++half) {
-      if (wr == half) {
-#pragma unroll
-        for (int i = 0; i < MT; ++i)
-#pragma unroll
-          for (int pr = 0; pr < 2; ++pr) {
-            const int row = i * 16 + l15;
-            const int chunk = (2 * pr + (lq & 1)) * 2 + (lq >> 1);
-            *(f16x8*)(ybuf + wc * E_REGION + row * 128 + ((chunk ^ (row & 7)) * 16)) = ykeep[i][pr];
-          }
-      }
-      asm volatile("s_waitcnt lgkmcnt(0)" ::: "memory");
-      __builtin_amdgcn_s_barrier();
-      f32x4 acc2[4][2];
-#pragma unroll
-      for (int i = 0; i < 4; ++i)
-#pragma unroll
-        for (int f = 0; f < 2; ++f) acc2[i][f] = f32x4{0.f, 0.f, 0.f, 0.f};
-#pragma unroll
-      for (int ks = 0; ks < 4; ++ks)
-#pragma unroll
-        for (int kh = 0; kh < 2; ++kh) {
-          f16x8 wf[2], yf[4];
-#pragma unroll
-          for (int f = 0; f < 2; ++f) wf[f] = *(const f16x8*)(wbuf + ks * E_REGION + ((fw + f * 2048) ^ (kh * 64)));
-#pragma unroll
-          for (int i = 0; i < 4; ++i) yf[i] = *(const f16x8*)(ybuf + ks * E_REGION + ((fy + i * 2048) ^ (kh * 64)));
-#pragma unroll
-          for (int i = 0; i < 4; ++i)
-#pragma unroll
-            for (int f = 0; f < 2; ++f) acc2[i][f] = __builtin_amdgcn_mfma_f32_16x16x32_f16(wf[f], yf[i], acc2[i][f], 0, 0, 0);
-        }
-      od_mfma_results_ready();
-      e8_epilogue_direct<4, 2>(p2, acc2, m0 + half * WROWS + rg * 64, cg * 32, l15, lq, nullptr, WROWS - rg * 64, sc2, bi2);
-      if (half == 0) {
-        asm volatile("s_waitcnt lgkmcnt(0)" ::: "memory");
-        __builtin_amdgcn_s_barrier();
-      }
-    }
-  } else if (p.splitk > 1) {
-    conv_epilogue<E_BN, 2, 4, MT, 4, 512>(p, smem, acc, m0, n0, tid, wr, wc, l15, lq);
-  } else {
-    od_mfma_results_ready();
-    e8_epilogue_direct<MT>(p, acc, m0 + wr * WROWS, n0 + wc * 64, l15, lq);
-  }
-}
-
 struct E8Entry {
   int BM;
-  const void* k1;
-  const char* name1;
-  const void* k1pw;
-  const void* k3pw;
-  const char* name1pw;
-  const char* name3pw;
-  const void* k3seg;
-  const char* name3seg;
+  bool (*variant)(int ksize, bool pw, int epi, int epi2, const void** fn, const char** name);
 };
-#define OD_E8(MF1)                                                                                                   \
-  {                                                                                                                  \
-    32 * (4 + MF1), (const void*)&od_conv_8ph<1, MF1>, "od_conv_8ph<1, " #MF1 ", false, false>",                     \
-        (const void*)&od_conv_8ph<1, MF1, true>, (const void*)&od_conv_8ph<3, MF1, true>,                            \
-        "od_conv_8ph<1, " #MF1 ", true, false>", "od_conv_8ph<3, " #MF1 ", true, false>",                            \
-        (const void*)&od_conv_8ph<3, MF1, false, true>, "od_conv_8ph<3, " #MF1 ", false, true>"                      \
-  }
-const E8Entry g_e8[] = {OD_E8(4), OD_E8(3), OD_E8(2), OD_E8(1)};
+const E8Entry g_e8[] = {{256, od_conv_8ph_variant_mf4}, {224, od_conv_8ph_variant_mf3}, {192, od_conv_8ph_variant_mf2},
+                        {160, od_conv_8ph_variant_mf1}};
 constexpr int kNumE8 = sizeof(g_e8) / sizeof(g_e8[0]);
 
 }
@@ -513,8 +28,13 @@
   const bool pw = p.w2 != nullptr;
   if (p.nseg > 1 && (ksize != 3 || pw || p.stride != 1 || p.res_mode != OD_RES_NONE)) return false;
   const size_t epi = (size_t)(e.BM / 2) * (E_BN + 4) * 4;
-  *info = {ksize == 1 ? (pw ? e.k1pw : e.k1) : (pw ? e.k3pw : e.k3seg),
-           ksize == 1 ? (pw ? e.name1pw : e.name1) : (pw ? e.name3pw : e.name3seg),
-           e.BM, E_BN, E_BK, 512, epi > (size_t)2 * E_BUF ? epi : (size_t)2 * E_BUF};
+  const int epi1 = od_epi_of(p);
+  const int epi2 = (pw && epi1 != OD_EPI_RT) ? od_epi(p.act2, OD_RES_NONE, false) : OD_EPI_RT;
+  const void* fn;
+  const char* name;
+  if (!e.variant(ksize, pw, epi1, epi2, &fn, &name) &&
+      !e.variant(ksize, pw, OD_EPI_RT, OD_EPI_RT, &fn, &name))
+    return false;
+  *info = {fn, name, e.BM, E_BN, E_BK, 512, epi > (size_t)2 * E_BUF ? epi : (size_t)2 * E_BUF};
   return true;
 }
diff --git a/object_detector_amd/csrc/conv_8ph_inst.hip b/object_detector_amd/csrc/conv_8ph_inst.hip
--- /dev/null
+++ b/object_detector_amd/csrc/conv_8ph_inst.hip
@@ -0,0 +1,51 @@
+#include "conv_8ph_kernel.h"
+
+#ifndef OD_E8_MF1
+#error "compile with -DOD_E8_MF1=1..4"
+#endif
+
+namespace {
+
+struct E8Variant {
+  int ksize;
+  bool pw;
+  int epi, epi2;
+  const void* fn;
+  const char* name;
+};
+#define OD_E8V(KS, PW, SEG, EPI, EPI2)                                                                                  \
+  {KS, PW, EPI, EPI2, (const void*)&od_conv_8ph<KS, OD_E8_MF1, EPI, EPI2, PW, SEG>,                                     \
+   "od_conv_8ph<" #KS ", " OD_STR(OD_E8_MF1) ", " OD_STR(EPI) ", " OD_STR(EPI2) ", " #PW ", " #SEG ">"}
+const E8Variant g_variants[] = {
+    OD_E8V(1, false, false, OD_EPI_RT, OD_EPI_RT),
+    OD_E8V(1, false, false, OD_EPI_LEAKY_NONE_F16, OD_EPI_RT),
+    OD_E8V(1, false, false, OD_EPI_ELU_NONE_F16, OD_EPI_RT),
+    OD_E8V(1, false, false, OD_EPI_ELU_UP2_F16, OD_EPI_RT),
+    OD_E8V(1, false, false, OD_EPI_ELU_NONE_F32, OD_EPI_RT),
+    OD_E8V(3, false, true, OD_EPI_RT, OD_EPI_RT),
+    OD_E8V(3, false, true, OD_EPI_LEAKY_NONE_F16, OD_EPI_RT),
+    OD_E8V(3, false, true, OD_EPI_LEAKY_SAME_F16, OD_EPI_RT),
+    OD_E8V(3, false, true, OD_EPI_ELU_NONE_F16, OD_EPI_RT),
+    OD_E8V(3, false, true, OD_EPI_ELU_UP2_F16, OD_EPI_RT),
+    OD_E8V(3, false, true, OD_EPI_LINEAR_NONE_F32, OD_EPI_RT),
+    OD_E8V(3, false, true, OD_EPI_LEAKY_NONE_F32, OD_EPI_RT),
+    OD_E8V(3, false, true, OD_EPI_ELU_NONE_F32, OD_EPI_RT),
+    OD_E8V(1, true, false, OD_EPI_RT, OD_EPI_RT),
+    OD_E8V(3, true, false, OD_EPI_RT, OD_EPI_RT),
+    OD_E8V(3, true, false, OD_EPI_LEAKY_NONE_F16, OD_EPI_LEAKY_NONE_F16),
+    OD_E8V(3, true, false, OD_EPI_LEAKY_SAME_F16, OD_EPI_LEAKY_NONE_F16),
+};
+
+}
+
+#define OD_CAT_(a, b) a##b
+#define OD_CAT(a, b) OD_CAT_(a, b)
+bool OD_CAT(od_conv_8ph_variant_mf, OD_E8_MF1)(int ksize, bool pw, int epi, int epi2, const void** fn, const char** name) {
+  for (const E8Variant& v : g_variants)
+    if (v.ksize == ksize && v.pw == pw && v.epi == epi && v.epi2 == epi2) {
+      *fn = v.fn;
+      *name = v.name;
+      return true;
+    }
+  return false;
+}
diff --git a/object_detector_amd/csrc/conv_8ph_kernel.h b/object_detector_amd/csrc/conv_8ph_kernel.h
--- /dev/null
+++ b/object_detector_amd/csrc/conv_8ph_kernel.h
@@ -0,0 +1,571 @@
+#pragma once
+#include "conv_8ph_tile.h"
+#include "conv_common.h"
+
+namespace {
+
+constexpr int E_ALO = 0, E_AHI = E_REGION, E_BLO = 2 * E_REGION, E_BHI = 3 * E_REGION;
+
+struct TapWalk {
+  int c0, tap, tapoff, dx;
+  int sel_tap;
+};
+
+constexpr unsigned E_OOB = 0x80000000u;
+
+template <int MT, int NF = 4, bool KEEP = false>
+static __device__ __forceinline__ void e8_epilogue_rt(const ConvKP& p, f32x4 (&acc)[MT][NF], int m0w, int n0w, int l15,
+                                                          int lq, f16x8 (*keep)[NF / 2] = nullptr, int mrows = MT * 16,
+                                                          const float* pre_sc = nullptr, const float* pre_bi = nullptr) {
+  unsigned pb[MT], ppix[MT];
+#pragma unroll
+  for (int i = 0; i < MT; ++i) {
+    const int m = m0w + i * 16 + l15;
+    pb[i] = (unsigned)m / (unsigned)p.HoWo;
+    ppix[i] = (unsigned)m - pb[i] * (unsigned)p.HoWo;
+  }
+#pragma unroll
+  for (int pr = 0; pr < NF / 2; ++pr) {
+    const int n = n0w + (2 * pr + (lq & 1)) * 16 + (lq >> 1) * 8;
+    const bool nok = n < p.Cout;
+    float sc[8], bi[8];
+    if (pre_sc) {
+#pragma unroll
+      for (int e = 0; e < 8; ++e) {
+        sc[e] = pre_sc[e];
+        bi[e] = pre_bi[e];
+      }
+    } else {
+      const f32x4 s0 = *(const f32x4*)(p.scale + n), s1 = *(const f32x4*)(p.scale + n + 4);
+      const f32x4 b0 = *(const f32x4*)(p.bias + n), b1 = *(const f32x4*)(p.bias + n + 4);
+#pragma unroll
+      for (int e = 0; e < 4; ++e) {
+        sc[e] = s0[e];
+        sc[4 + e] = s1[e];
+        bi[e] = b0[e];
+        bi[4 + e] = b1[e];
+      }
+    }
+    f16x8 rv[MT];
+#pragma unroll
+    for (int i = 0; i < MT; ++i) {
+      const int m = m0w + i * 16 + l15;
+      f16x8 r = {0, 0, 0, 0, 0, 0, 0, 0};
+      if (nok && m < p.M && p.res_mode != OD_RES_NONE) {
+        long long roff;
+        if (p.res_mode == OD_RES_SAME) {
+          roff = (long long)m * p.Cout + n;
+        } else {
+          const unsigned ho = ppix[i] / (unsigned)p.Wo, wo = ppix[i] - ho * (unsigned)p.Wo;
+          roff = ((long long)(pb[i] * (unsigned)(p.Ho >> 1) + (ho >> 1)) * (p.Wo >> 1) + (wo >> 1)) * p.Cout + n;
+        }
+        r = *(const f16x8*)(p.res + roff);
+      }
+      rv[i] = r;
+    }
+#pragma unroll
+    for (int i = 0; i < MT; ++i) {
+      const int m = m0w + i * 16 + l15;
+      const bool ok = nok && m < p.M && i * 16 + l15 < mrows;
+      float v[8];
+#pragma unroll
+      for (int e = 0; e < 4; ++e) {
+        float a = acc[i][2 * pr][e], bq = acc[i][2 * pr + 1][e];
+        od_permlane16_swap(a, bq);
+        v[e] = a;
+        v[4 + e] = bq;
+      }
+#pragma unroll
+      for (int e = 0; e < 8; ++e) v[e] = v[e] * sc[e] + bi[e];
+      if (p.act == OD_ACT_LEAKY) {
+#pragma unroll
+        for (int e = 0; e < 8; ++e) v[e] = od_leaky(v[e], p.alpha);
+      } else if (p.act == OD_ACT_ELU) {
+#pragma unroll
+        for (int e = 0; e < 8; ++e) v[e] = v[e] > 0.f ? v[e] : p.alpha * od_expm1_fast(v[e]);
+      }
+      if (p.res_mode != OD_RES_NONE) {
+#pragma unroll
+        for (int e = 0; e < 8; ++e) v[e] += (float)rv[i][e];
+      }
+      if (ok) {
+        const long long ooff = (long long)pb[i] * p.obs + (long long)ppix[i] * p.ops + n;
+        if (p.out_f32) {
+          float* o = (float*)p.out + ooff;
+          *(f32x4*)o = f32x4{v[0], v[1], v[2], v[3]};
+          *(f32x4*)(o + 4) = f32x4{v[4], v[5], v[6], v[7]};
+        } else {
+          f16x8 h;
+#pragma unroll
+          for (int e = 0; e < 8; ++e) h[e] = (f16)v[e];
+          *(f16x8*)((f16*)p.out + ooff) = h;
+        }
+      }
+      if (KEEP) {
+        f16x8 h;
+#pragma unroll
+        for (int e = 0; e < 8; ++e) h[e] = (f16)v[e];
+        keep[i][pr] = h;
+      }
+    }
+  }
+}
+
+template <int EPI, int MT, int NF, bool KEEP>
+static __device__ __forceinline__ void e8_epilogue_fixed(const ConvKP& p, f32x4 (&acc)[MT][NF], int m0w, int n0w, int l15, int lq,
+                                                         f16x8 (*keep)[NF / 2], int mrows, const float* pre_sc,
+                                                         const float* pre_bi) {
+  constexpr int ACT = od_epi_act(EPI), RES = od_epi_res(EPI);
+  constexpr bool F32 = od_epi_f32(EPI);
+  unsigned orow[MT], rrow[RES != OD_RES_NONE ? MT : 1];
+#pragma unroll
+  for (int i = 0; i < MT; ++i) {
+    const unsigned m = (unsigned)min(m0w + i * 16 + l15, p.M - 1);
+    const unsigned b = m / (unsigned)p.HoWo, pix = m - b * (unsigned)p.HoWo;
+    orow[i] = b * (unsigned)p.obs + pix * (unsigned)p.ops;
+    if (RES == OD_RES_SAME) rrow[i] = m * (unsigned)p.Cout;
+    if (RES == OD_RES_UP2) {
+      const unsigned ho = pix / (unsigned)p.Wo, wo = pix - ho * (unsigned)p.Wo;
+      rrow[i] = ((b * (unsigned)(p.Ho >> 1) + (ho >> 1)) * (unsigned)(p.Wo >> 1) + (wo >> 1)) * (unsigned)p.Cout;
+    }
+  }
+#pragma unroll
+  for (int pr = 0; pr < NF / 2; ++pr) {
+    const int n = n0w + (2 * pr + (lq & 1)) * 16 + (lq >> 1) * 8;
+    const bool nok = n < p.Cout;
+    float sc[8], bi[8];
+    if (pre_sc) {
+#pragma unroll
+      for (int e = 0; e < 8; ++e) {
+        sc[e] = pre_sc[e];
+        bi[e] = pre_bi[e];
+      }
+    } else {
+      const f32x4 s0 = *(const f32x4*)(p.scale + n), s1 = *(const f32x4*)(p.scale + n + 4);
+      const f32x4 b0 = *(const f32x4*)(p.bias + n), b1 = *(const f32x4*)(p.bias + n + 4);
+#pragma unroll
+      for (int e = 0; e < 4; ++e) {
+        sc[e] = s0[e];
+        sc[4 + e] = s1[e];
+        bi[e] = b0[e];
+        bi[4 + e] = b1[e];
+      }
+    }
+    f16x8 rv[RES != OD_RES_NONE ? MT : 1];
+    if (RES != OD_RES_NONE) {
+      const unsigned nr = nok ? (unsigned)n : 0u;
+#pragma unroll
+      for (int i = 0; i < MT; ++i) rv[i] = *(const f16x8*)(p.res + (rrow[i] + nr));
+    }
+#pragma unroll
+    for (int i = 0; i < MT; ++i) {
+      f32x4 a = acc[i][2 * pr], bq = acc[i][2 * pr + 1];
+      od_permlane16_swap4(a, bq);
+      float v[8] = {a[0], a[1], a[2], a[3], bq[0], bq[1], bq[2], bq[3]};
+#pragma unroll
+      for (int e = 0; e < 8; ++e) v[e] = v[e] * sc[e] + bi[e];
+      if (ACT == OD_ACT_LEAKY) {
+#pragma unroll
+        for (int e = 0; e < 8; ++e) v[e] = od_leaky(v[e], p.alpha);
+      } else if (ACT == OD_ACT_ELU) {
+#pragma unroll
+        for (int e = 0; e < 8; ++e) v[e] = od_elu_select(v[e], p.alpha);
+      }
+      if (RES != OD_RES_NONE) {
+#pragma unroll
+        for (int e = 0; e < 8; ++e) v[e] += (float)rv[i][e];
+      }
+      f16x8 h;
+      if (!F32 || KEEP) {
+#pragma unroll
+        for (int e = 0; e < 8; ++e) h[e] = (f16)v[e];
+      }
+      if (nok && m0w + i * 16 + l15 < p.M && i * 16 + l15 < mrows) {
+        const unsigned ooff = orow[i] + (unsigned)n;
+        if (F32) {
+          float* o = (float*)p.out + ooff;
+          *(f32x4*)o = f32x4{v[0], v[1], v[2], v[3]};
+          *(f32x4*)(o + 4) = f32x4{v[4], v[5], v[6], v[7]};
+        } else {
+          *(f16x8*)((f16*)p.out + ooff) = h;
+        }
+      }
+      if (KEEP) keep[i][pr] = h;
+    }
+  }
+}
+
+template <int MT, int NF = 4, bool KEEP = false, int EPI = OD_EPI_RT>
+static __device__ __forceinline__ void e8_epilogue_direct(const ConvKP& p, f32x4 (&acc)[MT][NF], int m0w, int n0w, int l15,
+                                                          int lq, f16x8 (*keep)[NF / 2] = nullptr, int mrows = MT * 16,
+                                                          const float* pre_sc = nullptr, const float* pre_bi = nullptr) {
+  if constexpr (EPI == OD_EPI_RT)
+    e8_epilogue_rt<MT, NF, KEEP>(p, acc, m0w, n0w, l15, lq, keep, mrows, pre_sc, pre_bi);
+  else
+    e8_epilogue_fixed<EPI, MT, NF, KEEP>(p, acc, m0w, n0w, l15, lq, keep, mrows, pre_sc, pre_bi);
+}
+
+template <int KS, int MF1, int EPI, int EPI2, bool PW, bool SEG>
+__global__ __launch_bounds__(512, 2) void od_conv_8ph(ConvKP p_in) {
+  constexpr int MF0 = 4, MT = MF0 + MF1, WROWS = MT * 16, BM = 2 * WROWS;
+  extern __shared__ __attribute__((aligned(16))) char smem[];
+  const int tid = threadIdx.x;
+  const int lane = tid & 63;
+  const int wave = __builtin_amdgcn_readfirstlane(tid >> 6);
+  const int wr = wave >> 2, wc = wave & 3;
+  const int l15 = lane & 15, lq = lane >> 4;
+
+  int logical;
+  {
+    const int nt = p_in.mtiles * p_in.ntiles;
+    const int pid = p_in.splitk > 1 ? (int)blockIdx.x / p_in.splitk : (int)blockIdx.x;
+    const int q = nt >> 3, r = nt & 7, xcd = pid & 7, loc = pid >> 3;
+    logical = (xcd < r ? xcd * (q + 1) : r * (q + 1) + (xcd - r) * q) + loc;
+  }
+  int tm = logical / p_in.ntiles;
+  const int tn = logical - tm * p_in.ntiles;
+  ConvKP p_seg;
+  if (SEG) p_seg = p_in;
+  if (SEG && p_in.nseg > 1) {
+    int sg = 0;
+    if (tm >= p_in.seg_tile0[1]) sg = 1;
+    if (p_in.nseg > 2 && tm >= p_in.seg_tile0[2]) sg = 2;
+    tm -= p_in.seg_tile0[sg];
+    p_seg.x = p_in.seg_x[sg];
+    p_seg.out = p_in.seg_out[sg];
+    p_seg.H = p_seg.Ho = p_in.seg_H[sg];
+    p_seg.W = p_seg.Wo = p_in.seg_W[sg];
+    p_seg.HoWo = p_seg.H * p_seg.W;
+    p_seg.M = p_in.seg_M[sg];
+    p_seg.x_bytes = (unsigned)p_seg.M * (unsigned)p_in.Cin * 2u;
+    if (p_in.obs == 0) p_seg.obs = (long long)p_seg.HoWo * p_in.Cout;
+  }
+  const ConvKP& p = SEG ? p_seg : p_in;
+  const int m0 = tm * BM, n0 = tn * E_BN;
+  const int nk_all = p.Ktot / E_BK;
+  const int ks0 = p.splitk > 1 ? ((int)blockIdx.x % p.splitk) * p.steps_per_split : 0;
+  const int nk = p.splitk > 1 ? min(p.steps_per_split, nk_all - ks0) : nk_all;
+  if (nk <= 0) return;
+
+  const int rr = tid >> 3;
+  const int lc = (tid & 7) ^ (rr & 7);
+  int a_base[2][2];
+  unsigned a_vmask[2][2];
+  unsigned a_sel[2][2];
+#pragma unroll
+  for (int s = 0; s < 2; ++s)
+#pragma unroll
+    for (int j = 0; j < 2; ++j) {
+      const int m = m0 + j * WROWS + s * 64 + rr;
+      a_vmask[s][j] = 0u;
+      a_base[s][j] = 0;
+      if (m < p.M && (s == 0 || rr < MF1 * 16)) {
+        const unsigned b = (unsigned)m / (unsigned)p.HoWo;
+        const unsigned pix = (unsigned)m - b * (unsigned)p.HoWo;
+        const unsigned ho = pix / (unsigned)p.Wo;
+        const unsigned wo = pix - ho * (unsigned)p.Wo;
+        const int hi0 = (int)ho * p.stride - p.pad, wi0 = (int)wo * p.stride - p.pad;
+        a_base[s][j] = ((((int)b * p.H + hi0 + p.pad) * p.W + wi0 + p.pad) * p.Cin + lc * 8) * 2;
+#pragma unroll
+        for (int t = 0; t < KS * KS; ++t) {
+          const int hi = hi0 + t / KS, wi = wi0 + t % KS;
+          if ((unsigned)hi < (unsigned)p.H && (unsigned)wi < (unsigned)p.W) a_vmask[s][j] |= 1u << t;
+        }
+      }
+    }
+  int w_off[2][2];
+#pragma unroll
+  for (int s = 0; s < 2; ++s)
+#pragma unroll
+    for (int j = 0; j < 2; ++j) {
+      const int n = n0 + (2 * j + (rr >> 5)) * 64 + s * 32 + (rr & 31);
+      w_off[s][j] = (n * p.Kstride + lc * 8 + ks0 * E_BK) * 2;
+    }
+  const __amdgpu_buffer_rsrc_t rs_x = __builtin_amdgcn_make_buffer_rsrc(
+      (void*)(p.x - (long long)p.pad * (p.W + 1) * p.Cin), 0, (int)(p.x_bytes + (unsigned)(p.pad * (p.W + 1) * p.Cin * 2)),
+      0x00020000);
+  const __amdgpu_buffer_rsrc_t rs_w = __builtin_amdgcn_make_buffer_rsrc((void*)p.w, 0, (int)p.w_bytes, 0x00020000);
+  auto blds16 = [&](const __amdgpu_buffer_rsrc_t& rs, unsigned voff, int soff, char* lptr) {
+    __builtin_amdgcn_raw_ptr_buffer_load_lds(rs, (__attribute__((address_space(3))) void*)lptr, 16, (int)voff, soff, 0, 0);
+  };
+
+  auto walk_init = [&](TapWalk& w, int kt) {
+    const int k0 = kt * E_BK;
+    if (KS == 3) {
+      w.sel_tap = -1;
+      w.tap = k0 / p.Cin;
+      w.c0 = k0 - w.tap * p.Cin;
+      const int dy = w.tap / 3;
+      w.dx = w.tap - dy * 3;
+      w.tapoff = (dy * p.W + w.dx) * p.Cin;
+    } else {
+      w.sel_tap = -1;
+      w.tap = 0;
+      w.c0 = k0;
+      w.dx = 0;
+      w.tapoff = 0;
+    }
+  };
+  auto walk_next = [&](TapWalk& w) {
+    w.c0 += E_BK;
+    if (KS == 3 && w.c0 >= p.Cin) {
+      w.c0 = 0;
+      ++w.tap;
+      if (++w.dx == 3) {
+        w.dx = 0;
+        w.tapoff += (p.W - 2) * p.Cin;
+      } else {
+        w.tapoff += p.Cin;
+      }
+    }
+  };
+  TapWalk walk_lo, walk_hi;
+  walk_init(walk_lo, ks0);
+  walk_init(walk_hi, ks0);
+
+  char* const piece = smem + wave * 1024;
+  auto stage_a = [&](int s, TapWalk& w, int buf) {
+    const int koff = w.tapoff + w.c0;
+    char* dst = piece + buf * E_BUF + (s ? E_AHI : E_ALO);
+    if (w.sel_tap != w.tap) {
+      w.sel_tap = w.tap;
+#pragma unroll
+      for (int j = 0; j < 2; ++j) a_sel[s][j] = ((a_vmask[s][j] >> w.tap) & 1u) ? (unsigned)a_base[s][j] : E_OOB;
+    }
+#pragma unroll
+    for (int j = 0; j < 2; ++j) blds16(rs_x, a_sel[s][j], koff * 2, dst + j * 8192);
+    walk_next(w);
+  };
+  auto stage_b = [&](int s, int t, int buf) {
+    char* dst = piece + buf * E_BUF + (s ? E_BHI : E_BLO);
+#pragma unroll
+    for (int j = 0; j < 2; ++j) blds16(rs_w, (unsigned)w_off[s][j], t * (E_BK * 2), dst + j * 8192);
+  };
+
+  const int w2buf = ((nk - 1) & 1) ^ 1;
+  const __amdgpu_buffer_rsrc_t rs_w2 =
+      __builtin_amdgcn_make_buffer_rsrc((void*)(PW ? p.w2 : p.w), 0, (int)(PW ? p.w2_bytes : p.w_bytes), 0x00020000);
+  auto stage_w2 = [&](int ks) {
+#pragma unroll
+    for (int h = 0; h < 2; ++h)
+      blds16(rs_w2, (unsigned)(((h * 64 + rr) * p.K2stride + lc * 8) * 2), ks * (E_BK * 2),
+             piece + w2buf * E_BUF + ks * E_REGION + h * 8192);
+  };
+
+  f32x4 acc[MT][4];
+#pragma unroll
+  for (int i = 0; i < MT; ++i)
+#pragma unroll
+    for (int j = 0; j < 4; ++j) acc[i][j] = f32x4{0.f, 0.f, 0.f, 0.f};
+
+  stage_a(0, walk_lo, 0);
+  stage_b(0, 0, 0);
+  stage_b(1, 0, 0);
+  stage_a(1, walk_hi, 0);
+  if (nk > 1) {
+    stage_a(0, walk_lo, 1);
+    stage_b(0, 1, 1);
+    wait_vmcnt<8>();
+  } else {
+    wait_vmcnt<0>();
+  }
+  __builtin_amdgcn_s_barrier();
+
+  const int fa = (wr * 64 + l15) * 128 + ((lq ^ (l15 & 7)) * 16);
+  const int fb = (wc * 32 + l15) * 128 + ((lq ^ (l15 & 7)) * 16);
+
+  f16x8 xa[MF0][2], wlo[2][2], whi[2][2];
+  auto ldf = [&](f16x8& dst, const char* src) { dst = *(const f16x8*)src; };
+  auto mma = [&](f32x4& c, const f16x8& a, const f16x8& b) {
+    c = __builtin_amdgcn_mfma_f32_16x16x32_f16(a, b, c, 0, 0, 0);
+  };
+
+  auto L0 = [&](int t) {
+    const char* cur = smem + (t & 1) * E_BUF;
+#pragma unroll
+    for (int f = 0; f < 2; ++f)
+#pragma unroll
+      for (int kh = 0; kh < 2; ++kh) ldf(wlo[f][kh], cur + E_BLO + ((fb + f * 2048) ^ (kh * 64)));
+#pragma unroll
+    for (int f = 0; f < MF0; ++f)
+#pragma unroll
+      for (int kh = 0; kh < 2; ++kh) ldf(xa[f][kh], cur + E_ALO + ((fa + f * 2048) ^ (kh * 64)));
+    if (t + 1 < nk) {
+      stage_b(1, t + 1, (t & 1) ^ 1);
+      wait_vmcnt<8>();
+    } else if (PW) {
+      stage_w2(0);
+      wait_vmcnt<2>();
+    } else {
+      wait_vmcnt<0>();
+    }
+  };
+  auto L1 = [&](int t) {
+    const char* cur = smem + (t & 1) * E_BUF;
+#pragma unroll
+    for (int f = 0; f < 2; ++f)
+#pragma unroll
+      for (int kh = 0; kh < 2; ++kh) ldf(whi[f][kh], cur + E_BHI + ((fb + f * 2048) ^ (kh * 64)));
+    if (t + 1 < nk) {
+      stage_a(1, walk_hi, (t & 1) ^ 1);
+      wait_vmcnt<8>();
+    } else if (PW) {
+      stage_w2(1);
+    } else {
+      wait_vmcnt<0>();
+    }
+  };
+  auto L2 = [&](int t) {
+    const char* cur = smem + (t & 1) * E_BUF;
+#pragma unroll
+    for (int f = 0; f < MF1; ++f)
+#pragma unroll
+      for (int kh = 0; kh < 2; ++kh) ldf(xa[f][kh], cur + E_AHI + ((fa + f * 2048) ^ (kh * 64)));
+    if (t + 2 < nk) stage_a(0, walk_lo, t & 1);
+    if (PW && t + 1 == nk) stage_w2(2);
+  };
+  auto L3 = [&](int t) {
+    if (t + 2 < nk) {
+      stage_b(0, t + 2, t & 1);
+      wait_vmcnt<8>();
+    } else if (PW && t + 1 == nk) {
+      stage_w2(3);
+    } else {
+      wait_vmcnt<0>();
+    }
+  };
+  auto M = [&](int ph) {
+    __builtin_amdgcn_s_setprio(1);
+#pragma unroll
+    for (int kh = 0; kh < 2; ++kh)
+#pragma unroll
+      for (int i = 0; i < ((ph < 2) ? MF0 : MF1); ++i)
+#pragma unroll
+        for (int j = 0; j < 2; ++j) {
+          if (ph == 0) mma(acc[i][j], wlo[j][kh], xa[i][kh]);
+          if (ph == 1) mma(acc[i][2 + j], whi[j][kh], xa[i][kh]);
+          if (ph == 2) mma(acc[MF0 + i][2 + j], whi[j][kh], xa[i][kh]);
+          if (ph == 3) mma(acc[MF0 + i][j], wlo[j][kh], xa[i][kh]);
+        }
+    __builtin_amdgcn_s_setprio(0);
+  };
+
+  if (wr == 0) {
+    for (int t = 0; t < nk; ++t) {
+      L0(t);
+      M(0);
+      __builtin_amdgcn_s_barrier();
+      L1(t);
+      M(1);
+      __builtin_amdgcn_s_barrier();
+      L2(t);
+      M(2);
+      __builtin_amdgcn_s_barrier();
+      L3(t);
+      M(3);
+      __builtin_amdgcn_s_barrier();
+    }
+  } else {
+    L0(0);
+    __builtin_amdgcn_s_barrier();
+    for (int t = 0; t < nk; ++t) {
+      M(0);
+      L1(t);
+      __builtin_amdgcn_s_barrier();
+      M(1);
+      L2(t);
+      __builtin_amdgcn_s_barrier();
+      M(2);
+      L3(t);
+      __builtin_amdgcn_s_barrier();
+      M(3);
+      if (t + 1 < nk) {
+        L0(t + 1);
+        __builtin_amdgcn_s_barrier();
+      }
+    }
+  }
+  __syncthreads();
+
+  if constexpr (PW) {
+    const int rg = wave >> 2, cg = wave & 3;
+    float sc2[8], bi2[8];
+    {
+      const int n2 = cg * 32 + (lq & 1) * 16 + (lq >> 1) * 8;
+      const f32x4 s0 = *(const f32x4*)(p.scale2 + n2), s1 = *(const f32x4*)(p.scale2 + n2 + 4);
+      const f32x4 b0 = *(const f32x4*)(p.bias2 + n2), b1 = *(const f32x4*)(p.bias2 + n2 + 4);
+#pragma unroll
+      for (int e = 0; e < 4; ++e) {
+        sc2[e] = s0[e];
+        sc2[4 + e] = s1[e];
+        bi2[e] = b0[e];
+        bi2[4 + e] = b1[e];
+      }
+    }
+    f16x8 ykeep[MT][2];
+    od_mfma_results_ready();
+    e8_epilogue_direct<MT, 4, true, EPI>(p, acc, m0 + wr * WROWS, n0 + wc * 64, l15, lq, ykeep);
+    ConvKP p2 = p;
+    p2.scale = p.scale2;
+    p2.bias = p.bias2;
+    p2.act = p.act2;
+    p2.alpha = p.alpha2;
+    p2.res_mode = OD_RES_NONE;
+    p2.out = (void*)p.out2;
+    p2.out_f32 = 0;
+    p2.Cout = p.Cout2;
+    p2.obs = (long long)p.HoWo * p.Cout2;
+    p2.ops = p.Cout2;
+    char* const ybuf = smem + (w2buf ^ 1) * E_BUF;
+    const char* const wbuf = smem + w2buf * E_BUF;
+    const int fy = (rg * 64 + l15) * 128 + ((lq ^ (l15 & 7)) * 16);
+    const int fw = (cg * 32 + l15) * 128 + ((lq ^ (l15 & 7)) * 16);
+#pragma unroll
+    for (int half = 0; half < 2; ++half) {
+      if (wr == half) {
+#pragma unroll
+        for (int i = 0; i < MT; ++i)
+#pragma unroll
+          for (int pr = 0; pr < 2; ++pr) {
+            const int row = i * 16 + l15;
+            const int chunk = (2 * pr + (lq & 1)) * 2 + (lq >> 1);
+            *(f16x8*)(ybuf + wc * E_REGION + row * 128 + ((chunk ^ (row & 7)) * 16)) = ykeep[i][pr];
+          }
+      }
+      asm volatile("s_waitcnt lgkmcnt(0)" ::: "memory");
+      __builtin_amdgcn_s_barrier();
+      f32x4 acc2[4][2];
+#pragma unroll
+      for (int i = 0; i < 4; ++i)
+#pragma unroll
+        for (int f = 0; f < 2; ++f) acc2[i][f] = f32x4{0.f, 0.f, 0.f, 0.f};
+#pragma unroll
+      for (int ks = 0; ks < 4; ++ks)
+#pragma unroll
+        for (int kh = 0; kh < 2; ++kh) {
+          f16x8 wf[2], yf[4];
+#pragma unroll
+          for (int f = 0; f < 2; ++f) wf[f] = *(const f16x8*)(wbuf + ks * E_REGION + ((fw + f * 2048) ^ (kh * 64)));
+#pragma unroll
+          for (int i = 0; i < 4; ++i) yf[i] = *(const f16x8*)(ybuf + ks * E_REGION + ((fy + i * 2048) ^ (kh * 64)));
+#pragma unroll
+          for (int i = 0; i < 4; ++i)
+#pragma unroll
+            for (int f = 0; f < 2; ++f) acc2[i][f] = __builtin_amdgcn_mfma_f32_16x16x32_f16(wf[f], yf[i], acc2[i][f], 0, 0, 0);
+        }
+      od_mfma_results_ready();
+      e8_epilogue_direct<4, 2, false, EPI2>(p2, acc2, m0 + half * WROWS + rg * 64, cg * 32, l15, lq, nullptr, WROWS - rg * 64, sc2, bi2);
+      if (half == 0) {
+        asm volatile("s_waitcnt lgkmcnt(0)" ::: "memory");
+        __builtin_amdgcn_s_barrier();
+      }
+    }
+  } else if (EPI == OD_EPI_RT && p.splitk > 1) {
+    conv_epilogue<E_BN, 2, 4, MT, 4, 512>(p, smem, acc, m0, n0, tid, wr, wc, l15, lq);
+  } else {
+    od_mfma_results_ready();
+    e8_epilogue_direct<MT, 4, false, EPI>(p, acc, m0 + wr * WROWS, n0 + wc * 64, l15, lq);
+  }
+}
+
+}
diff --git a/object_detector_amd/csrc/conv_8ph_tile.h b/object_detector_amd/csrc/conv_8ph_tile.h
--- /dev/null
+++ b/object_detector_amd/csrc/conv_8ph_tile.h
@@ -0,0 +1,9 @@
+#pragma once
+
+namespace {
+
+constexpr int E_BN = 256, E_BK = 64;
+constexpr int E_REGION = 128 * 128;
+constexpr int E_BUF = 4 * E_REGION;
+
+}
diff --git a/object_detector_amd/csrc/conv_common.h b/object_detector_amd/csrc/conv_common.h
--- a/object_detector_amd/csrc/conv_common.h
+++ b/object_detector_amd/csrc/conv_common.h
@@ -36,6 +36,7 @@
   const f16* seg_x[3];
   void* seg_out[3];
   int seg_H[3], seg_W[3], seg_M[3];
+  int off32;
 };
 
 static __device__ __forceinline__ void glds16(const void* gptr, void* lptr) {
@@ -48,8 +49,51 @@
   return v > -0.25f ? poly : __expf(v) - 1.f;
 }
 
+static __device__ __forceinline__ float od_elu_select(float v, float alpha) {
+  const float poly = v * (1.f + v * (0.5f + v * (1.f / 6 + v * (1.f / 24 + v * (1.f / 120 + v * (1.f / 720))))));
+  const float ex = __expf(v) - 1.f;
+  const float em = v > -0.25f ? poly : ex;
+  const float neg = alpha * em;
+  return v > 0.f ? v : neg;
+}
+
+#define OD_EPI_RT -1
+#define OD_EPI_LEAKY_NONE_F16 1
+#define OD_EPI_LEAKY_SAME_F16 5
+#define OD_EPI_ELU_NONE_F16 2
+#define OD_EPI_ELU_UP2_F16 10
+#define OD_EPI_LINEAR_NONE_F32 16
+#define OD_EPI_LEAKY_NONE_F32 17
+#define OD_EPI_ELU_NONE_F32 18
+constexpr int od_epi(int act, int res_mode, bool out_f32) { return act | (res_mode << 2) | ((int)out_f32 << 4); }
+static_assert(od_epi(OD_ACT_LEAKY, OD_RES_NONE, false) == OD_EPI_LEAKY_NONE_F16 &&
+                  od_epi(OD_ACT_LEAKY, OD_RES_SAME, false) == OD_EPI_LEAKY_SAME_F16 &&
+                  od_epi(OD_ACT_ELU, OD_RES_NONE, false) == OD_EPI_ELU_NONE_F16 &&
+                  od_epi(OD_ACT_ELU, OD_RES_UP2, false) == OD_EPI_ELU_UP2_F16 &&
+                  od_epi(OD_ACT_LINEAR, OD_RES_NONE, true) == OD_EPI_LINEAR_NONE_F32 &&
+                  od_epi(OD_ACT_LEAKY, OD_RES_NONE, true) == OD_EPI_LEAKY_NONE_F32 &&
+                  od_epi(OD_ACT_ELU, OD_RES_NONE, true) == OD_EPI_ELU_NONE_F32,
+              "OD_EPI_* literals");
+constexpr int od_epi_act(int epi) { return epi & 3; }
+constexpr int od_epi_res(int epi) { return (epi >> 2) & 3; }
+constexpr bool od_epi_f32(int epi) { return ((epi >> 4) & 1) != 0; }
+static inline int od_epi_of(const ConvKP& p) {
+  return (p.off32 && p.splitk <= 1 && !p.tconv && !p.stats) ? od_epi(p.act, p.res_mode, p.out_f32 != 0) : OD_EPI_RT;
+}
+#define OD_STR_(x) #x
+#define OD_STR(x) OD_STR_(x)
+
 static __device__ __forceinline__ void od_permlane16_swap(float& a, float& b) {
   asm volatile("s_nop 1\n\tv_permlane16_swap_b32 %0, %1\n\ts_nop 1" : "+v"(a), "+v"(b));
+}
+static __device__ __forceinline__ void od_permlane16_swap4(f32x4& a, f32x4& b) {
+  float a0 = a[0], a1 = a[1], a2 = a[2], a3 = a[3], b0 = b[0], b1 = b[1], b2 = b[2], b3 = b[3];
+  asm volatile(
+      "s_nop 1\n\tv_permlane16_swap_b32 %0, %4\n\tv_permlane16_swap_b32 %1, %5\n\tv_permlane16_swap_b32 %2, %6\n\t"
+      "v_permlane16_swap_b32 %3, %7\n\ts_nop 1"
+      : "+v"(a0), "+v"(a1), "+v"(a2), "+v"(a3), "+v"(b0), "+v"(b1), "+v"(b2), "+v"(b3));
+  a = f32x4{a0, a1, a2, a3};
+  b = f32x4{b0, b1, b2, b3};
 }
 static __device__ __forceinline__ void od_mfma_results_ready() {
   __builtin_amdgcn_sched_barrier(0);
@@ -75,10 +119,15 @@
   return (int)(b * (unsigned)p.HoWo + (2u * i + (cls >> 1)) * (unsigned)p.Wo + 2u * j + (cls & 1u));
 }
 
-template <int BN, int WM, int WN, int MT, int NTL, int NT = WM * WN * 64, bool STATS = false>
+template <int BN, int WM, int WN, int MT, int NTL, int NT = WM * WN * 64, bool STATS = false, int EPI = OD_EPI_RT>
 static __device__ __forceinline__ void conv_epilogue(const ConvKP& p, char* smem, f32x4 (&acc)[MT][NTL], int m0, int n0,
                                                      int tid, int wm, int wn, int l15, int lq) {
   constexpr int WTM = MT * 16, WTN = NTL * 16, SLD = BN + 4;
+  constexpr bool FX = EPI != OD_EPI_RT;
+  static_assert(!(FX && STATS), "the statistics epilogue has no policy");
+  const int act = FX ? od_epi_act(EPI) : p.act, res_mode = FX ? od_epi_res(EPI) : p.res_mode;
+  const bool out_f32 = FX ? od_epi_f32(EPI) : p.out_f32 != 0;
+  const bool splitk = !FX && p.splitk > 1, tconv = !FX && p.tconv;
   float* stg = (float*)smem;
   constexpr int CH = BN / 8;
   constexpr int RPP = NT / CH;
@@ -104,7 +153,7 @@
   constexpr int NPASS = (WTM + RPP - 1) / RPP;
   constexpr bool RAGGED = (WTM % RPP) != 0;
   f16x8 resv[WM][NPASS];
-  if (p.res_mode != OD_RES_NONE && p.splitk <= 1) {
+  if (res_mode != OD_RES_NONE && !splitk) {
 #pragma unroll
     for (int wr = 0; wr < WM; ++wr)
 #pragma unroll
@@ -112,10 +161,10 @@
         int m = m0 + wr * WTM + ps * RPP + tid / CH;
         f16x8 r = {0, 0, 0, 0, 0, 0, 0, 0};
         if (RAGGED && ps * RPP + tid / CH >= WTM) m = p.M;
-        if (p.tconv && m < p.M) m = od_tconv_pixel(p, (unsigned)m, WM * MT * 16);
+        if (tconv && m < p.M) m = od_tconv_pixel(p, (unsigned)m, WM * MT * 16);
         if (m >= 0 && m < p.M && n < p.Cout) {
           long long roff;
-          if (p.res_mode == OD_RES_SAME) {
+          if (res_mode == OD_RES_SAME) {
             roff = (long long)m * p.Cout + n;
           } else {
             const unsigned b = (unsigned)m / (unsigned)p.HoWo;
@@ -139,7 +188,7 @@
       }
     }
     __syncthreads();
-    if (p.splitk > 1) {
+    if (splitk) {
       float* slab = p.ws + (long long)((int)blockIdx.x % p.splitk) * p.M * p.Cout;
 #pragma unroll
       for (int ps = 0; ps < NPASS; ++ps) {
@@ -158,7 +207,7 @@
     for (int ps = 0; ps < NPASS; ++ps) {
       const int row = ps * RPP + tid / CH;
       int m = (RAGGED && row >= WTM) ? p.M : m0 + wr * WTM + row;
-      if (p.tconv && m < p.M) m = od_tconv_pixel(p, (unsigned)m, WM * MT * 16);
+      if (tconv && m < p.M) m = od_tconv_pixel(p, (unsigned)m, WM * MT * 16);
       if (m >= 0 && m < p.M && n < p.Cout) {
         const f32x4 v0 = *(const f32x4*)(stg + row * SLD + c8);
         const f32x4 v1 = *(const f32x4*)(stg + row * SLD + c8 + 4);
@@ -168,21 +217,22 @@
           for (int e = 0; e < 8; ++e) v[e] = v[e] * sc[e] + bi[e];
         }
         if (STATS) {
-        } else if (p.act == OD_ACT_LEAKY) {
+        } else if (act == OD_ACT_LEAKY) {
 #pragma unroll
           for (int e = 0; e < 8; ++e) v[e] = od_leaky(v[e], p.alpha);
-        } else if (p.act == OD_ACT_ELU) {
-#pragma unroll
-          for (int e = 0; e < 8; ++e) v[e] = v[e] > 0.f ? v[e] : p.alpha * od_expm1_fast(v[e]);
-        }
-        if (!STATS && p.res_mode != OD_RES_NONE) {
+        } else if (act == OD_ACT_ELU) {
+#pragma unroll
+          for (int e = 0; e < 8; ++e) v[e] = FX ? od_elu_select(v[e], p.alpha) : (v[e] > 0.f ? v[e] : p.alpha * od_expm1_fast(v[e]));
+        }
+        if (!STATS && res_mode != OD_RES_NONE) {
 #pragma unroll
           for (int e = 0; e < 8; ++e) v[e] += (float)resv[wr][ps][e];
         }
         const unsigned b = (unsigned)m / (unsigned)p.HoWo;
         const unsigned pix = (unsigned)m - b * (unsigned)p.HoWo;
-        const long long ooff = (long long)b * p.obs + (long long)pix * p.ops + n;
-        if (p.out_f32) {
+        const long long ooff = FX ? (long long)(b * (unsigned)p.obs + pix * (unsigned)p.ops + (unsigned)n)
+                                  : (long long)b * p.obs + (long long)pix * p.ops + n;
+        if (out_f32) {
           float* o = (float*)p.out + ooff;
           *(f32x4*)o = f32x4{v[0], v[1], v[2], v[3]};
           *(f32x4*)(o + 4) = f32x4{v[4], v[5], v[6], v[7]};
@@ -254,13 +304,17 @@
 };
 
 int od_conv_igemm_num_cfgs();
-bool od_conv_igemm_select(int cfg, int ksize, int Cin, bool want_stats, ConvKernelInfo* info);
+bool od_conv_igemm_select(int cfg, int ksize, int Cin, bool want_stats, int epi, ConvKernelInfo* info);
 int od_conv_finish_prepare(const ConvKP& p, od_launches* L);
 int od_conv_8ph_num_cfgs();
 long od_conv_8ph_tiles(int idx, int M, int Cout);
 double od_conv_8ph_tile_cost(int idx, int nk);
 bool od_conv_8ph_can_fuse_pointwise(const ConvKP& p);
 bool od_conv_8ph_select(int idx, const ConvKP& p, int ksize, ConvKernelInfo* info);
+bool od_conv_8ph_variant_mf4(int ksize, bool pw, int epi, int epi2, const void** fn, const char** name);
+bool od_conv_8ph_variant_mf3(int ksize, bool pw, int epi, int epi2, const void** fn, const char** name);
+bool od_conv_8ph_variant_mf2(int ksize, bool pw, int epi, int epi2, const void** fn, const char** name);
+bool od_conv_8ph_variant_mf1(int ksize, bool pw, int epi, int epi2, const void** fn, const char** name);
 bool od_tconv_small_supported(const od_conv_desc* d);
 int od_tconv_small_prepare(od_ctx* ctx, const od_conv_desc* d, od_launches* L);
 bool od_conv_rdirect_supported(const od_conv_desc* d);
diff --git a/object_detector_amd/csrc/conv_dispatch.hip b/object_detector_amd/csrc/conv_dispatch.hip
--- a/object_detector_amd/csrc/conv_dispatch.hip
+++ b/object_detector_amd/csrc/conv_dispatch.hip
@@ -147,6 +147,10 @@
   p.w_bytes = (unsigned)((long long)od_round_up(d->Cout, 256) * p.Kstride * 2);
   p.obs = d->out_batch_stride ? d->out_batch_stride : (long long)p.HoWo * d->Cout;
   p.ops = d->out_pix_stride ? d->out_pix_stride : d->Cout;
+  long long hw_max = p.HoWo;
+  for (int i = 0; grouped && i < d->nseg; ++i) hw_max = hw_max > (long long)d->seg_H[i] * d->seg_W[i] ? hw_max : (long long)d->seg_H[i] * d->seg_W[i];
+  p.off32 = p.obs >= 0 && p.ops >= 0 && (long long)d->B * p.obs < (1LL << 31) &&
+            (long long)(d->B - 1) * p.obs + (hw_max - 1) * p.ops + d->Cout < (1LL << 31);
   p.splitk = 1;
   p.steps_per_split = 0;
   p.ws = (float*)d->splitk_workspace;
@@ -172,7 +176,7 @@
     od_set_error("od_conv2d_fwd: tile_cfg %d (8-phase kernel) needs Cin %% 64 == 0 and no transposed gather", cfg);
     return OD_ERR_INVALID;
   }
-  if (od_conv_igemm_select(cfg, d->ksize, d->Cin, want_stats, k)) return OD_OK;
+  if (od_conv_igemm_select(cfg, d->ksize, d->Cin, want_stats, od_epi_of(p), k)) return OD_OK;
   od_set_error("od_conv2d_fwd: tile_cfg %d needs Cin %% %d == 0 for 3x3 (Cin = %d); use cfg 0-3", cfg, k->BK, d->Cin);
   return OD_ERR_INVALID;
 }
@@ -257,10 +261,8 @@
       p.splitk = od_ceil_div(nk, p.steps_per_split);
     }
   }
-  if (d->w2 && use_e8 && od_conv_8ph_can_fuse_pointwise(p)) {
-    p.w2 = (const f16*)d->w2;
-    if (int rc = conv_select(cfg, d, p, want_stats, &k)) return rc;
-  }
+  if (d->w2 && use_e8 && od_conv_8ph_can_fuse_pointwise(p)) p.w2 = (const f16*)d->w2;
+  if (int rc = conv_select(cfg, d, p, want_stats, &k)) return rc;
   if (int rc = od_ensure_lds(ctx, k.fn, k.lds)) return rc;
   const size_t launch_lds = (use_e8 && p.splitk <= 1 && k.lds > (size_t)128 * 1024) ? (size_t)128 * 1024 : k.lds;
   if (int rc = od_add_launch(L, {k.name, od_issue_kp, k.fn, dim3(p.mtiles * p.ntiles * p.splitk), dim3(k.threads), launch_lds}, p))
diff --git a/object_detector_amd/csrc/conv_mfma.hip b/object_detector_amd/csrc/conv_mfma.hip
--- a/object_detector_amd/csrc/conv_mfma.hip
+++ b/object_detector_amd/csrc/conv_mfma.hip
@@ -26,7 +26,8 @@
   static_assert(LOADS * (STAGES - 2 > 0 ? STAGES - 2 : 0) <= 63, "vmcnt field");
 };
 
-template <int BM, int BN, int BK, int STAGES, int WM, int WN, int KS, int MINW, bool UNI, int SPEC, bool STATS = false>
+template <int BM, int BN, int BK, int STAGES, int WM, int WN, int KS, int MINW, bool UNI, int SPEC, bool STATS = false,
+          int EPI = OD_EPI_RT>
 __global__ __launch_bounds__(WM* WN * 64 * (SPEC ? 2 : 1), MINW) void od_conv_igemm(ConvKP p) {
   using Cf = ConvCfg<BM, BN, BK, STAGES, WM, WN, SPEC>;
   constexpr int NT = Cf::NT, AR = Cf::AR, BR = Cf::BR, RPR = Cf::RPR, ROWB = Cf::ROWB;
@@ -268,7 +269,7 @@
   }
   __syncthreads();
 
-  conv_epilogue<BN, WM, WN, MT, NTL, Cf::NTHREADS, STATS>(p, smem, acc, m0, n0, tid_all, is_consumer ? wm : -1, wn, l15, lq);
+  conv_epilogue<BN, WM, WN, MT, NTL, Cf::NTHREADS, STATS, EPI>(p, smem, acc, m0, n0, tid_all, is_consumer ? wm : -1, wn, l15, lq);
 }
 
 __global__ __launch_bounds__(256) void od_conv_finish(ConvKP p) {
@@ -325,18 +326,29 @@
   int BM, BN, BK, threads;
   size_t lds;
   struct { const void* fn; const char* name; } k[3][2];
+  struct { const void* fn; const char* name; } fx[2][4];
 };
+constexpr int kFxEpi[4] = {OD_EPI_LEAKY_NONE_F16, OD_EPI_LEAKY_SAME_F16, OD_EPI_ELU_NONE_F16, OD_EPI_ELU_UP2_F16};
 
 #define OD_K1(BM, BN, BK, ST, WM, WN, KS, MINW, UNI, SPEC, STATS)                                                       \
   {(const void*)&od_conv_igemm<BM, BN, BK, ST, WM, WN, KS, MINW, UNI, SPEC, STATS>,                                     \
-   "od_conv_igemm<" #BM ", " #BN ", " #BK ", " #ST ", " #WM ", " #WN ", " #KS ", " #MINW ", " #UNI ", " #SPEC ", " #STATS ">"}
+   "od_conv_igemm<" #BM ", " #BN ", " #BK ", " #ST ", " #WM ", " #WN ", " #KS ", " #MINW ", " #UNI ", " #SPEC ", " #STATS ", -1>"}
+#define OD_KX1(BM, BN, BK, ST, WM, WN, KS, MINW, UNI, SPEC, EPI)                                                         \
+  {(const void*)&od_conv_igemm<BM, BN, BK, ST, WM, WN, KS, MINW, UNI, SPEC, false, EPI>,                                \
+   "od_conv_igemm<" #BM ", " #BN ", " #BK ", " #ST ", " #WM ", " #WN ", " #KS ", " #MINW ", " #UNI ", " #SPEC ", false, " OD_STR(EPI) ">"}
+#define OD_KX(BM, BN, BK, ST, WM, WN, KS, MINW, UNI, SPEC)                                                             \
+  {OD_KX1(BM, BN, BK, ST, WM, WN, KS, MINW, UNI, SPEC, OD_EPI_LEAKY_NONE_F16),                                          \
+   OD_KX1(BM, BN, BK, ST, WM, WN, KS, MINW, UNI, SPEC, OD_EPI_LEAKY_SAME_F16),                                          \
+   OD_KX1(BM, BN, BK, ST, WM, WN, KS, MINW, UNI, SPEC, OD_EPI_ELU_NONE_F16),                                            \
+   OD_KX1(BM, BN, BK, ST, WM, WN, KS, MINW, UNI, SPEC, OD_EPI_ELU_UP2_F16)}
 #define OD_K(BM, BN, BK, ST, WM, WN, KS, MINW, UNI, SPEC)                                                              \
   {OD_K1(BM, BN, BK, ST, WM, WN, KS, MINW, UNI, SPEC, false), OD_K1(BM, BN, BK, ST, WM, WN, KS, MINW, UNI, SPEC, true)}
 #define OD_NOK(BM, BN, BK, ST, WM, WN, KS, MINW, UNI, SPEC) {}
 #define OD_CFG(BM, BN, BK, ST, WM, WN, MINW, SPEC, K3G)                                                                 \
   {BM, BN, BK, WM * WN * 64 * (SPEC + 1), (size_t)ConvCfg<BM, BN, BK, ST, WM, WN, SPEC>::LDS_BYTES,                     \
    {OD_K(BM, BN, BK, ST, WM, WN, 1, MINW, true, SPEC), OD_K(BM, BN, BK, ST, WM, WN, 3, MINW, true, SPEC),               \
-    K3G(BM, BN, BK, ST, WM, WN, 3, MINW, false, SPEC)}}
+    K3G(BM, BN, BK, ST, WM, WN, 3, MINW, false, SPEC)},                                                                 \
+   {OD_KX(BM, BN, BK, ST, WM, WN, 1, MINW, true, SPEC), OD_KX(BM, BN, BK, ST, WM, WN, 3, MINW, true, SPEC)}}
 
 const TileCfg g_cfgs[] = {
     OD_CFG(128, 128, 64, 2, 2, 2, 2, 0, OD_K),
@@ -354,12 +366,18 @@
 
 int od_conv_igemm_num_cfgs() { return kNumCfgs; }
 
-bool od_conv_igemm_select(int cfg, int ksize, int Cin, bool want_stats, ConvKernelInfo* info) {
+bool od_conv_igemm_select(int cfg, int ksize, int Cin, bool want_stats, int epi, ConvKernelInfo* info) {
   if (cfg < 0 || cfg >= kNumCfgs) return false;
   const TileCfg& tc = g_cfgs[cfg];
-  const auto& k = tc.k[ksize == 1 ? 0 : ((Cin % tc.BK) == 0 ? 1 : 2)][want_stats];
+  const int var = ksize == 1 ? 0 : ((Cin % tc.BK) == 0 ? 1 : 2);
+  const auto& k = tc.k[var][want_stats];
   *info = {k.fn, k.name, tc.BM, tc.BN, tc.BK, tc.threads, tc.lds};
-  return k.fn != nullptr;
+  for (int i = 0; i < 4 && var < 2 && !want_stats; ++i)
+    if (kFxEpi[i] == epi) {
+      info->fn = tc.fx[var][i].fn;
+      info->name = tc.fx[var][i].name;
+    }
+  return info->fn != nullptr;
 }
 
 int od_conv_finish_prepare(const ConvKP& p, od_launches* L) {
```

New measurement: 22280, median of 6. +3.3%, better.
